# Eawag-SIAM/SimulatedAnnealingABC.jl

Hardware: AMD Instinct MI355X
Metric: particle-simulations/sec at n_particles=1e6 (higher is better)
Workload: dtype f64

## Files before the change

### include/sabc_hip.h

```cpp
#ifndef SABC_HIP_H
#define SABC_HIP_H

#include <stdint.h>

#ifdef __cplusplus
extern "C" {
#endif

#define SABC_ABI_VERSION 6
#define SABC_MAX_PARA 16
#define SABC_MAX_STATS 64
#define SABC_MAX_SOURCE_STATS 64
#define SABC_MAX_JOINT_PARA 8
#define SABC_MAX_MODEL_PARAMS 32

#if defined(__GNUC__)
#define SABC_API __attribute__((visibility("default")))
#else
#define SABC_API
#endif

enum { SABC_MODEL_HOST = 0,
       SABC_MODEL_GAUSS_IID = 1, SABC_MODEL_GAUSS2D = 2, SABC_MODEL_GK = 3, SABC_MODEL_LV = 4,
       SABC_MODEL_USER = 5     };
// ... 115 lines not shown
SABC_API int64_t     sabc_comm_p2p_fallbacks(const sabc_handle *h);
SABC_API int         sabc_comm_p2p_inject_silence(sabc_handle *h, int32_t n);
SABC_API int         sabc_comm_p2p_inject_loss(sabc_handle *h, int32_t n);
SABC_API int         sabc_comm_p2p_inject_stale(sabc_handle *h, int32_t n);

SABC_API int sabc_initialize(sabc_handle *h, int64_t n_simulation);
SABC_API int sabc_update(sabc_handle *h, const sabc_update_args *args);

SABC_API int64_t sabc_n_global(const sabc_handle *h);
SABC_API int64_t sabc_n_local(const sabc_handle *h);
SABC_API int64_t sabc_local_offset(const sabc_handle *h);
SABC_API int sabc_get_population(sabc_handle *h, double *theta, double *u, double *rho);
SABC_API int sabc_set_population(sabc_handle *h, const double *theta, const double *u, const double *rho);
SABC_API int sabc_get_counters(const sabc_handle *h, int64_t out[4]);
SABC_API int sabc_set_counters(sabc_handle *h, const int64_t in[4]);
SABC_API int sabc_get_epsilon(const sabc_handle *h, double *eps, int32_t *len);
SABC_API int sabc_set_epsilon(sabc_handle *h, const double *eps, int32_t len);
SABC_API int64_t sabc_history_len(const sabc_handle *h);
SABC_API int sabc_get_history(const sabc_handle *h, double *eps_hist, double *u_hist, double *rho_hist);
SABC_API int sabc_clear_history(sabc_handle *h);
SABC_API int64_t sabc_cdf_len(const sabc_handle *h, int32_t stat);
SABC_API int sabc_get_cdf_knots(sabc_handle *h, int32_t stat, double *out);
SABC_API int sabc_set_cdf_knots(sabc_handle *h, int32_t stat, const double *knots, int64_t len);
SABC_API int sabc_cdf_apply(sabc_handle *h, const double *rho, int64_t m, double *u_out);
SABC_API int sabc_get_proposal_sigma(const sabc_handle *h, double *sigma_dxd);
SABC_API double sabc_last_ess(const sabc_handle *h);

SABC_API int sabc_op_build_cdf(int32_t device, const double *x, int64_t n, double *knots_out, int64_t *len_out);
SABC_API int sabc_op_cdf_eval(int32_t device, const double *knots, int64_t len, const double *q, int64_t m,
                              double *out);
SABC_API int sabc_op_sort(int32_t device, const double *x, int64_t n, double *out);
SABC_API int sabc_op_eps_single(double ubar, double v, double *eps_out);
SABC_API int sabc_op_eps_multi(const double *ubar, int32_t s, double v, double *eps_out);
SABC_API int sabc_op_simulate(sabc_handle *h, const double *theta, int64_t m, uint64_t pid0, uint64_t iter,
                              double *rho_out);
SABC_API int sabc_op_prior(sabc_handle *h, uint64_t pid0, int64_t m, double *theta_out, double *logpdf_out);
SABC_API int sabc_op_philox(int32_t device, uint64_t seed, uint64_t pid, uint32_t purpose, uint64_t iter, uint32_t k,
                            uint32_t out_words[4], double out_normals[2]);

SABC_API int sabc_op_normal_pairs(int32_t device, uint64_t seed, uint64_t pid0, uint32_t purpose, uint64_t iter,
                                  uint32_t k, int64_t m, double *out_2m);

SABC_API int sabc_op_rng_peak(int32_t device, int64_t n_lanes, int32_t pairs_per_lane, int32_t repeats,
                              double *normals_per_s);

enum { SABC_KERNEL_UPDATE = 0, SABC_KERNEL_REDUCE = 1, SABC_KERNEL_RESAMPLE = 2, SABC_KERNEL_INIT = 3,
       SABC_KERNEL_COLLECTIVE = 4,
       SABC_KERNEL_COUNT = 5 };
SABC_API int sabc_profile_enable(sabc_handle *h, int32_t level);
SABC_API int sabc_profile_get(sabc_handle *h, int32_t kernel, double *total_ms, int64_t *launches);
SABC_API int64_t sabc_profile_noops(sabc_handle *h, int32_t kernel);
SABC_API int64_t sabc_host_syncs(const sabc_handle *h);
SABC_API int64_t sabc_kernel_launches(const sabc_handle *h);
SABC_API int64_t sabc_persistent_launches(const sabc_handle *h);
SABC_API int32_t sabc_persistent_lanes(const sabc_handle *h);
SABC_API int64_t sabc_persistent_fallbacks(const sabc_handle *h);
SABC_API int64_t sabc_collective_calls(const sabc_handle *h);

#ifdef __cplusplus
}
#endif
#endif
```

### simulatedannealingabc.jl_amd/_lib.py

```python
from __future__ import annotations

import ctypes as C
import os
import subprocess

_HERE = os.path.dirname(os.path.abspath(__file__))
CSRC = os.path.join(_HERE, "csrc")
LIB_PATH = os.path.join(_HERE, "libsabc_hip.so")
HEADER = os.path.normpath(os.path.join(_HERE, "..", "include", "sabc_hip.h"))

ABI_VERSION = 6
P2P_DESC_BYTES, P2P_MAX_WORLD = 512, 8
MAX_PARA, MAX_STATS, MAX_MODEL_PARAMS = 16, 64, 32
MAX_SOURCE_STATS = 64
MAX_JOINT_PARA = 8
MODEL_HOST, MODEL_GAUSS_IID, MODEL_GAUSS2D, MODEL_GK, MODEL_LV, MODEL_USER = 0, 1, 2, 3, 4, 5
PRIOR_NORMAL, PRIOR_UNIFORM, PRIOR_EXPONENTIAL, PRIOR_LOGNORMAL, PRIOR_GAMMA, PRIOR_BETA, PRIOR_TRUNCNORMAL = 0, 1, 2, 3, 4, 5, 6
PROP_RANDOMWALK, PROP_DIFFEVO, PROP_STRETCH = 0, 1, 2
ALG_SINGLE_EPS, ALG_MULTI_EPS = 0, 1
KERNEL_UPDATE, KERNEL_REDUCE, KERNEL_RESAMPLE, KERNEL_INIT, KERNEL_COLLECTIVE = 0, 1, 2, 3, 4

ERR_NAMES = {
    -1: "NSIM_TOO_SMALL", -2: "NEG_DISTANCE", -3: "BAD_V", -4: "BAD_DELTA", -5: "BAD_ALGORITHM", -6: "BAD_BETA",
    -7: "ZERO_MEAN_U", -8: "BAD_CONFIG", -9: "NOT_POSDEF", -10: "EMPTY_CDF", -11: "ROOT", -20: "NO_DEVICE",
# ... 100 lines not shown
        "sabc_last_error": ([vp], C.c_char_p),
        "sabc_set_stream": ([vp, vp], C.c_int),
        "sabc_set_collectives": ([vp, ALLREDUCE_FN, ALLGATHER_FN, vp, C.c_int], C.c_int),
        "sabc_set_alltoallv": ([vp, ALLTOALLV_FN], C.c_int),
        "sabc_comm_bytes": ([vp], C.c_int64),
        "sabc_set_host_simulator": ([vp, SIMULATE_FN, vp], C.c_int),
        "sabc_set_host_prior": ([vp, PRIOR_SAMPLE_FN, PRIOR_LOGPDF_FN, vp], C.c_int),
        "sabc_register_device_simulator": ([vp, C.c_char_p], C.c_int),
        "sabc_op_compile_device_simulator": ([C.c_char_p, C.c_int32, C.c_int32, C.c_char_p, C.c_int64], C.c_int),
        "sabc_op_compile_device_simulator_with_prior": ([C.c_char_p, C.c_int32, C.c_int32, C.c_char_p, C.c_int64], C.c_int),
        "sabc_comm_init_rccl": ([vp, vp], C.c_int),
        "sabc_comm_unique_id": ([vp], C.c_int),
        "sabc_comm_selftest": ([vp], C.c_int),
        "sabc_initialize": ([vp, C.c_int64], C.c_int),
        "sabc_update": ([vp, C.POINTER(UpdateArgs)], C.c_int),
        "sabc_n_global": ([vp], C.c_int64),
        "sabc_n_local": ([vp], C.c_int64),
        "sabc_local_offset": ([vp], C.c_int64),
        "sabc_get_population": ([vp, dp, dp, dp], C.c_int),
        "sabc_set_population": ([vp, dp, dp, dp], C.c_int),
        "sabc_get_counters": ([vp, ip64], C.c_int),
        "sabc_set_counters": ([vp, ip64], C.c_int),
        "sabc_get_epsilon": ([vp, dp, C.POINTER(C.c_int32)], C.c_int),
        "sabc_set_epsilon": ([vp, dp, C.c_int32], C.c_int),
        "sabc_history_len": ([vp], C.c_int64),
        "sabc_get_history": ([vp, dp, dp, dp], C.c_int),
        "sabc_clear_history": ([vp], C.c_int),
        "sabc_cdf_len": ([vp, C.c_int32], C.c_int64),
        "sabc_get_cdf_knots": ([vp, C.c_int32, dp], C.c_int),
        "sabc_set_cdf_knots": ([vp, C.c_int32, dp, C.c_int64], C.c_int),
        "sabc_cdf_apply": ([vp, dp, C.c_int64, dp], C.c_int),
        "sabc_get_proposal_sigma": ([vp, dp], C.c_int),
        "sabc_last_ess": ([vp], C.c_double),
        "sabc_op_build_cdf": ([C.c_int32, dp, C.c_int64, dp, ip64], C.c_int),
        "sabc_op_sort": ([C.c_int32, dp, C.c_int64, dp], C.c_int),
        "sabc_op_cdf_eval": ([C.c_int32, dp, C.c_int64, dp, C.c_int64, dp], C.c_int),
        "sabc_op_eps_single": ([C.c_double, C.c_double, dp], C.c_int),
        "sabc_op_eps_multi": ([dp, C.c_int32, C.c_double, dp], C.c_int),
        "sabc_op_simulate": ([vp, dp, C.c_int64, C.c_uint64, C.c_uint64, dp], C.c_int),
        "sabc_op_prior": ([vp, C.c_uint64, C.c_int64, dp, dp], C.c_int),
        "sabc_op_philox": ([C.c_int32, C.c_uint64, C.c_uint64, C.c_uint32, C.c_uint64, C.c_uint32,
                            C.POINTER(C.c_uint32), dp], C.c_int),
        "sabc_op_normal_pairs": ([C.c_int32, C.c_uint64, C.c_uint64, C.c_uint32, C.c_uint64, C.c_uint32, C.c_int64, dp],
                                 C.c_int),
        "sabc_op_rng_peak": ([C.c_int32, C.c_int64, C.c_int32, C.c_int32, dp], C.c_int),
        "sabc_profile_enable": ([vp, C.c_int32], C.c_int),
        "sabc_profile_get": ([vp, C.c_int32, dp, ip64], C.c_int),
        "sabc_profile_noops": ([vp, C.c_int32], C.c_int64),
        "sabc_set_host_chunk": ([vp, C.c_int64], C.c_int),
        "sabc_host_callback_seconds": ([vp], C.c_double),
        "sabc_host_callback_calls": ([vp], C.c_int64),
        "sabc_host_syncs": ([vp], C.c_int64),
        "sabc_kernel_launches": ([vp], C.c_int64),
        "sabc_persistent_launches": ([vp], C.c_int64),
        "sabc_persistent_lanes": ([vp], C.c_int32),
        "sabc_persistent_fallbacks": ([vp], C.c_int64),
        "sabc_collective_calls": ([vp], C.c_int64),
        "sabc_comm_p2p_setup": ([vp], C.c_int),
        "sabc_comm_p2p_descriptor": ([vp, vp], C.c_int),
        "sabc_comm_p2p_init": ([vp, vp], C.c_int),
        "sabc_comm_p2p_selftest": ([vp], C.c_int),
        "sabc_comm_p2p_set_timeout": ([vp, C.c_double], C.c_int),
        "sabc_comm_p2p_disable": ([vp], C.c_int),
        "sabc_comm_p2p_active": ([vp], C.c_int),
        "sabc_comm_p2p_fallbacks": ([vp], C.c_int64),
        "sabc_comm_p2p_inject_silence": ([vp, C.c_int32], C.c_int),
        "sabc_comm_p2p_inject_stale": ([vp, C.c_int32], C.c_int),
        "sabc_comm_p2p_inject_loss": ([vp, C.c_int32], C.c_int),
        "sabc_comm_p2p_set_destroy_wait": ([vp, C.c_double], C.c_int),
        "sabc_comm_p2p_parked_bytes": ([], C.c_int64),
    }
    for name, (args, res) in sig.items():
        if not strict and not hasattr(L, name):
            continue
        fn = getattr(L, name)
        fn.argtypes, fn.restype = args, res
    return L


def global_error() -> str:
    return lib().sabc_last_global_error().decode("utf-8", "replace")
```

### simulatedannealingabc.jl_amd/csrc/capi.hip

```cpp
#include <hip/hip_runtime.h>
#include <dlfcn.h>

#include <cstdio>
#include <cstdlib>
#include <cstring>
#include <mutex>
#include <new>
#include <string>
#include <vector>

#include "../../include/sabc_hip.h"
#include "engine.hpp"
#include "hip_backend.hpp"
#include "host_math.hpp"
#include "kernels.hpp"
#include "p2p.hpp"
#include "p2p_setup.hpp"
#include "rtc.hpp"

using namespace sabc;

namespace {

thread_local std::string g_err;
// ... 622 lines not shown
  if (e == hipSuccess) e = hipMalloc((void **)&z, 16);
  if (e == hipSuccess) e = (hipError_t)launch_philox_debug(seed, pid, purpose, iter, k, w, z, nullptr);
  if (e == hipSuccess) e = hipMemcpy(out_words, w, 16, hipMemcpyDeviceToHost);
  if (e == hipSuccess) e = hipMemcpy(out_normals, z, 16, hipMemcpyDeviceToHost);
  (void)hipFree(w); (void)hipFree(z);
  if (e != hipSuccess) { g_err = hipGetErrorString(e); return SABC_ERR_HIP; }
  return 0;
}

int sabc_op_normal_pairs(int32_t device, uint64_t seed, uint64_t pid0, uint32_t purpose, uint64_t iter, uint32_t k,
                         int64_t m, double *out_2m) {
  std::string why;
  int rc = usable_device(device, why);
  if (rc) { g_err = why; return rc; }
  if (m <= 0) return 0;
  if (hipSetDevice(device) != hipSuccess) { g_err = "hipSetDevice failed"; return SABC_ERR_HIP; }
  double *d = nullptr;
  hipError_t e = hipMalloc((void **)&d, (size_t)m * 16);
  if (e == hipSuccess) e = (hipError_t)launch_normal_pairs(seed, pid0, purpose, iter, k, m, d, nullptr);
  if (e == hipSuccess) e = hipMemcpy(out_2m, d, (size_t)m * 16, hipMemcpyDeviceToHost);
  (void)hipFree(d);
  if (e != hipSuccess) { g_err = hipGetErrorString(e); return SABC_ERR_HIP; }
  return 0;
}

int sabc_op_rng_peak(int32_t device, int64_t n_lanes, int32_t pairs_per_lane, int32_t repeats, double *normals_per_s) {
  std::string why;
  int rc = usable_device(device, why);
  if (rc) { g_err = why; return rc; }
  if (n_lanes < 1 || pairs_per_lane < 1 || repeats < 1) { g_err = "bad arguments"; return SABC_ERR_BAD_CONFIG; }
  if (hipSetDevice(device) != hipSuccess) { g_err = "hipSetDevice failed"; return SABC_ERR_HIP; }
  double *d = nullptr;
  hipEvent_t a = nullptr, b = nullptr;
  hipError_t e = hipMalloc((void **)&d, (size_t)n_lanes * 8);
  if (e == hipSuccess) e = hipEventCreate(&a);
  if (e == hipSuccess) e = hipEventCreate(&b);
  if (e == hipSuccess) e = (hipError_t)launch_rng_peak(1, pairs_per_lane, n_lanes, d, nullptr);
  if (e == hipSuccess) e = hipEventRecord(a, nullptr);
  for (int r = 0; r < repeats && e == hipSuccess; ++r) e = (hipError_t)launch_rng_peak(2 + r, pairs_per_lane, n_lanes, d, nullptr);
  if (e == hipSuccess) e = hipEventRecord(b, nullptr);
  if (e == hipSuccess) e = hipEventSynchronize(b);
  float ms = 0.f;
  if (e == hipSuccess) e = hipEventElapsedTime(&ms, a, b);
  if (a) (void)hipEventDestroy(a);
  if (b) (void)hipEventDestroy(b);
  (void)hipFree(d);
  if (e != hipSuccess) { g_err = hipGetErrorString(e); return SABC_ERR_HIP; }
  *normals_per_s = 2.0 * (double)pairs_per_lane * (double)n_lanes * (double)repeats / ((double)ms * 1e-3);
  return 0;
}

int64_t sabc_host_syncs(const sabc_handle *h) { return h ? h->eng->host_syncs() : 0; }
int64_t sabc_kernel_launches(const sabc_handle *h) { return h ? h->be->kernel_launches() : 0; }
int64_t sabc_collective_calls(const sabc_handle *h) { return h ? h->eng->collective_calls() : 0; }

int sabc_profile_enable(sabc_handle *h, int32_t on) {
  if (!h) return SABC_ERR_STATE;
  h->be->profile_enable(on);
  return 0;
}

int64_t sabc_profile_noops(sabc_handle *h, int32_t kernel) { return h ? h->be->profile_noops(kernel) : 0; }

int sabc_profile_get(sabc_handle *h, int32_t kernel, double *total_ms, int64_t *launches) {
  if (!h) return SABC_ERR_STATE;
  return h->be->profile_get(kernel, total_ms, launches) ? hfail(h, SABC_ERR_HIP) : 0;
}

}
```

### simulatedannealingabc.jl_amd/csrc/device_models.hpp

```cpp
#pragma once
#include "device_rng.hpp"
#include "prior_math.hpp"
#include "kernels.hpp"
#include "sabc_types.hpp"

#ifndef SABC_GK_BLOCKMAX
#define SABC_GK_BLOCKMAX 1
#endif

namespace sabc {

#define SABC_LOG2PI 1.8378770664093454835606594728112

__device__ __forceinline__ double prior_logpdf_dim(const ModelDesc &m, int k, double x) {
  const int kind = m.prior_kind[k];
  const double a = m.prior_a[k], b = m.prior_b[k], lc = m.prior_logc[k];
  if (kind == SABC_PRIOR_NORMAL) {
    const double z = (x - a) / b;
    return -(z * z + SABC_LOG2PI) / 2.0 - lc;
  }
  if (kind == SABC_PRIOR_UNIFORM) return (x >= a && x <= b) ? -lc : -INFINITY;
  if (kind == SABC_PRIOR_EXPONENTIAL) return x >= 0.0 ? -x / a - lc : -INFINITY;
  if (kind == SABC_PRIOR_LOGNORMAL) {
    if (!(x > 0.0)) return -INFINITY;
// ... 302 lines not shown
  return cdf_interp(T, len, lo, x);
}

template <int N>
__device__ __forceinline__ void cdf_apply_mid_lockstep(const double *__restrict__ T, int64_t len, const double *__restrict__ M,
                                                       const double *x, double *u) {
  const int64_t mcount = (len + 15) >> kCdfLineShift;
  int64_t top = 1;
  while (top < mcount) top <<= 1;
  int64_t a[N];
#pragma unroll
  for (int p = 0; p < N; ++p) a[p] = 0;
  for (int64_t step = top >> 1; step >= 1; step >>= 1) {
#pragma unroll
    for (int p = 0; p < N; ++p) {
      const int64_t q = a[p] + step;
      const int64_t qs = q < mcount ? q : mcount - 1;
      const double v = M[qs];
      a[p] = (q < mcount && v < x[p]) ? q : a[p];
    }
  }
#pragma unroll
  for (int p = 0; p < N; ++p) a[p] <<= kCdfLineShift;
#pragma unroll
  for (int step = 1 << kCdfLineShift >> 1; step >= 1; step >>= 1) {
#pragma unroll
    for (int p = 0; p < N; ++p) a[p] += (T[a[p] + step] < x[p]) ? step : 0;
  }
  const double first = T[0], last = T[len - 1], L1 = (double)(len - 1);
  double t0[N], t1[N];
  int64_t i0[N];
#pragma unroll
  for (int p = 0; p < N; ++p) {
    const int64_t lo = first < x[p] ? a[p] + 1 : 0;
    i0[p] = lo > 0 ? lo - 1 : 0;
    t0[p] = T[i0[p]]; t1[p] = T[i0[p] + 1];
  }
#pragma unroll
  for (int p = 0; p < N; ++p) {
    const double y0 = (double)i0[p] / L1, y1 = (double)(i0[p] + 1) / L1;
    const double t = (x[p] - t0[p]) / (t1[p] - t0[p]);
    const double v = y0 + t * (y1 - y0);
    u[p] = !(x[p] >= first) ? ((x[p] != x[p]) ? x[p] : 0.0) : (x[p] > last ? 1.0 : v);
  }
}

__device__ __forceinline__ double finite_or_big(double v) { return isfinite(v) ? v : 1e30; }

template <int MODEL, int D, int S>
struct Sim;

template <int D, int S>
struct Sim<SABC_MODEL_GAUSS_IID, D, S> {
  static __device__ __forceinline__ void run(const ModelDesc &m, const double *th, uint64_t pid, uint64_t iter,
                                             double *rho, int coop = 0) {
    const int n_obs = (int)m.p[0];
    const double mu = th[0];
    const double sd = (D >= 2) ? th[1] : m.p[1];
    NormalStream ns(m.seed, pid, PURPOSE_SIM, iter, coop);
    double sz = 0.0, szz = 0.0;
    const int n_pairs = n_obs >> 1;
    ns.for_pairs(n_pairs, [&](const double z0, const double z1) {
      sz += z0; if (S >= 2) szz = fma(z0, z0, szz);
      sz += z1; if (S >= 2) szz = fma(z1, z1, szz);
    });
    if (n_obs & 1) {
      double z0, z1;
      ns.pair(z0, z1);
      sz += z0; if (S >= 2) szz = fma(z0, z0, szz);
    }
    const double n = (double)n_obs;
    rho[0] = fabs(m.p[2] - (mu + sd * sz / n));
    if (S >= 2) rho[1] = fabs(m.p[3] - (mu * mu + (2.0 * mu * sd * sz + sd * sd * szz) / n));
  }
};

template <int D, int S>
struct Sim<SABC_MODEL_GAUSS2D, D, S> {
  static __device__ __forceinline__ void run(const ModelDesc &m, const double *th, uint64_t pid, uint64_t iter,
                                             double *rho, int coop = 0) {
    const int n_obs = (int)m.p[0];
    const double r = m.p[1], c = sqrt(1.0 - r * r);
    NormalStream ns(m.seed, pid, PURPOSE_SIM, iter, coop);
    double A = 0, B = 0, AA = 0, BB = 0, AB = 0;
    ns.for_pairs(n_obs, [&](const double za, const double zb) {
      A += za; B += zb; AA = fma(za, za, AA); BB = fma(zb, zb, BB); AB = fma(za, zb, AB);
    });
    const double S1 = A, S2 = r * A + c * B;
    const double Q11 = AA, Q22 = r * r * AA + 2.0 * r * c * AB + c * c * BB, Q12 = r * AA + c * AB;
    const double m1 = S1 / n_obs, m2 = S2 / n_obs;
    const double var1 = (Q11 - S1 * m1) / (n_obs - 1), var2 = (Q22 - S2 * m2) / (n_obs - 1);
    const double cov = (Q12 - S1 * m2) / (n_obs - 1);
    const double d1 = th[0] + m1 - m.p[2], d2 = th[1] + m2 - m.p[3];
    rho[0] = sqrt(d1 * d1 + d2 * d2);
    if (S >= 2) rho[1] = fabs(var1 + var2 - m.p[4]);
    if (S >= 3) rho[2] = fabs(cov - m.p[5]);
  }
};

#if !defined(__HIPCC_RTC__)
constexpr int kGkMaxDraws = 128;
#ifndef SABC_GK_PW
#define SABC_GK_PW 64
#endif
constexpr int kGkParticlesPerWave = SABC_GK_PW;

__device__ __forceinline__ double gk_quantile(const double *th, double c, double z) {
  const double w = exp_tab(-0.5 * th[3] * neg2_log_tab(fma(z, z, 1.0)));
  return th[0] + th[1] * (1.0 + c * tanh_abs_tab(th[2] * z / 2.0)) * w * z;
}

template <int DIST>
__device__ __forceinline__ double xor_lane(double v) {
  int lo = __double2loint(v), hi = __double2hiint(v);
  if constexpr (DIST == 1) {
    lo = __builtin_amdgcn_mov_dpp(lo, 0xB1, 0xF, 0xF, true);
    hi = __builtin_amdgcn_mov_dpp(hi, 0xB1, 0xF, 0xF, true);
  } else if constexpr (DIST == 2) {
    lo = __builtin_amdgcn_mov_dpp(lo, 0x4E, 0xF, 0xF, true);
    hi = __builtin_amdgcn_mov_dpp(hi, 0x4E, 0xF, 0xF, true);
  } else if constexpr (DIST <= 16) {
    constexpr int pattern = 0x1F | (DIST << 10);
    lo = __builtin_amdgcn_ds_swizzle(lo, pattern);
    hi = __builtin_amdgcn_ds_swizzle(hi, pattern);
  } else {
    return __shfl_xor(v, DIST, 64);
  }
  return __hiloint2double(hi, lo);
}

template <int DIST>
__device__ __forceinline__ void half_swap(double &a, double &b) {
  static_assert(DIST == 16 || DIST == 32, "row-pair or half-wave swap");
  unsigned alo = (unsigned)__double2loint(a), ahi = (unsigned)__double2hiint(a);
  unsigned blo = (unsigned)__double2loint(b), bhi = (unsigned)__double2hiint(b);
  if constexpr (DIST == 32) {
    const auto l = __builtin_amdgcn_permlane32_swap(alo, blo, false, false);
    const auto h = __builtin_amdgcn_permlane32_swap(ahi, bhi, false, false);
    alo = l[0]; blo = l[1]; ahi = h[0]; bhi = h[1];
  } else {
    const auto l = __builtin_amdgcn_permlane16_swap(alo, blo, false, false);
    const auto h = __builtin_amdgcn_permlane16_swap(ahi, bhi, false, false);
    alo = l[0]; blo = l[1]; ahi = h[0]; bhi = h[1];
  }
  a = __hiloint2double((int)ahi, (int)alo);
  b = __hiloint2double((int)bhi, (int)blo);
}

constexpr uint64_t lane_bit(int i) {
// ... 171 lines not shown
  for (int i = 0; i < 8; ++i) v[i] = __hiloint2double(__double2hiint(v[i]) ^ sign_mask, __double2loint(v[i]));
}

template <int S>
__device__ __forceinline__ void gk_simulate_rows4(const ModelDesc &m, const double (*thp_lds)[4], double (*rp_lds)[S], const int my,
                                                  const uint64_t pid, const uint64_t iter) {
  const int lane = threadIdx.x & 63, rl = lane & 15;
  const int n_draws = (int)m.p[0];
  const double c = m.p[1];
  double th[4];
#pragma unroll
  for (int k = 0; k < 4; ++k) th[k] = thp_lds[my][k];
  const bool inc = gk_increasing(th, c);
  double v[8];
#pragma unroll
  for (int t = 0; t < 4; ++t) box_muller(stream_block(m.seed, pid, PURPOSE_SIM, iter, (uint32_t)(4 * rl + t)), v[2 * t], v[2 * t + 1]);
  if (!inc) {
#pragma unroll
    for (int i = 0; i < 8; ++i) v[i] = gk_quantile(th, c, v[i]);
  }
#pragma unroll
  for (int i = 0; i < 8; ++i) v[i] = 8 * rl + i < n_draws ? v[i] : INFINITY;
  const int b0 = (lane & 1) << 31, b1 = (lane & 2) << 30, b2 = (lane & 4) << 29, b3 = (lane & 8) << 28;
  gk_local_step<0, 1>(v);
  gk_local_step<1, 2>(v); gk_local_step<0, 2>(v);
  gk_flip(v, b0);
  gk_local_step<2, -1>(v); gk_local_step<1, -1>(v); gk_local_step<0, -1>(v);
  gk_flip(v, b1); gk_cross_step<1>(v);
  gk_flip(v, b0); gk_local_step<2, -1>(v); gk_local_step<1, -1>(v); gk_local_step<0, -1>(v);
  gk_flip(v, b2); gk_cross_step<2>(v);
  gk_flip(v, b1 ^ b0); gk_cross_step<1>(v);
  gk_flip(v, b0); gk_local_step<2, -1>(v); gk_local_step<1, -1>(v); gk_local_step<0, -1>(v);
  gk_flip(v, b3); gk_cross_step<4>(v);
  gk_flip(v, b2 ^ b1); gk_cross_step<2>(v);
  gk_flip(v, b1 ^ b0); gk_cross_step<1>(v);
  gk_flip(v, b0); gk_local_step<2, -1>(v); gk_local_step<1, -1>(v); gk_local_step<0, -1>(v);
  gk_cross_step<8>(v);
  gk_flip(v, b3 ^ b2); gk_cross_step<4>(v);
  gk_flip(v, b2 ^ b1); gk_cross_step<2>(v);
  gk_flip(v, b1);
  double bm = gk_max(gk_max(gk_max(v[0], v[1]), gk_max(v[2], v[3])), gk_max(gk_max(v[4], v[5]), gk_max(v[6], v[7])));
  bm = gk_max(bm, xor_lane<1>(bm));
#pragma unroll
  for (int j = 0; j < S; ++j) {
    const int lane_of_block = (((int)m.p[2 + j] >> 4) - 1) * 2;
    if (rl == lane_of_block) rp_lds[my][j] = inc ? bm : finite_or_big(fabs(bm - m.p[2 + S + j]));
  }
}

#endif

template <int D, int S>
struct Sim<SABC_MODEL_LV, D, S> {
  static __device__ __forceinline__ void run(const ModelDesc &m, const double *th, uint64_t pid, uint64_t iter,
                                             double *rho, int coop = 0) {
    const int n_steps = (int)m.p[0];
    const double dt = m.p[1], sg = m.p[2];
    double X = m.p[3], Y = m.p[4];
    const double sdt = sg * sqrt(dt);
    NormalStream ns(m.seed, pid, PURPOSE_SIM, iter, coop);
    double SX = 0, QX = 0, SY = 0, QY = 0;
    ns.for_pairs(n_steps, [&](const double z1, const double z2) {
      const double fx = fma(sdt, z1, fma(-th[1], Y, th[0]) * dt);
      const double fy = fma(sdt, z2, fma(th[1], X, -th[2]) * dt);
      X = fmax(fma(X, fx, X), 0.0);
      Y = fmax(fma(Y, fy, Y), 0.0);
      SX += X; QX += X * X; SY += Y; QY += Y * Y;
    });
    const double mX = SX / n_steps, mY = SY / n_steps;
    const double vX = (QX - SX * mX) / (n_steps - 1), vY = (QY - SY * mY) / (n_steps - 1);
    const double st[4] = {mX, sqrt(fmax(vX, 0.0)), mY, sqrt(fmax(vY, 0.0))};
#pragma unroll
    for (int j = 0; j < S; ++j) rho[j] = finite_or_big(fabs(st[j < 4 ? j : 3] - m.p[5 + j]));
  }
};

}
```

### simulatedannealingabc.jl_amd/csrc/device_rng.hpp

```cpp
#pragma once
#if !defined(__HIPCC_RTC__)
#include <hip/hip_runtime.h>
#endif
#include <stdint.h>
#ifndef INFINITY
#define INFINITY (__builtin_huge_val())
#endif

namespace sabc {

enum : uint32_t { PURPOSE_PRIOR = 0, PURPOSE_SIM = 1, PURPOSE_PROP = 2, PURPOSE_PROP2 = 3, PURPOSE_ACCEPT = 4,
                  PURPOSE_RESAMPLE = 5 };

struct u32x4 { uint32_t x, y, z, w; };

#if defined(__has_builtin)
#if __has_builtin(__builtin_amdgcn_bitop3_b32) && !defined(SABC_NO_BITOP3)
#define SABC_HAVE_BITOP3 1
#endif
#endif
__device__ __forceinline__ uint32_t xor3(uint32_t a, uint32_t b, uint32_t c) {
#if defined(SABC_HAVE_BITOP3)
  return __builtin_amdgcn_bitop3_b32(a, b, c, 0x96);
#else
// ... 260 lines not shown
}

__device__ __forceinline__ void box_muller(const u32x4 w, double &z0, double &z1, const Regs &c) {
  const double ua = loop::u52(w.x, w.y, c);
  const double ub = loop::u52(w.z, w.w, c);
  const double r = sqrt_fast(loop::neg2_log_tab(ua));
  double sn, cs;
  loop::sincos_2pi_tab(ub, sn, cs, c);
  z0 = r * cs;
  z1 = r * sn;
}

}

template <int W, int J>
__device__ __forceinline__ double team_pick_ct(const double v) {
  static_assert((W == 4 || W == 16) && J >= 0 && J < W, "a quad or a row of 16 lanes");
  constexpr int ctrl = W == 4 ? J * 0x55 : 0x150 + J;
  const int lo = __builtin_amdgcn_update_dpp(0, __double2loint(v), ctrl, 0xF, 0xF, true);
  const int hi = __builtin_amdgcn_update_dpp(0, __double2hiint(v), ctrl, 0xF, 0xF, true);
  return __hiloint2double(hi, lo);
}
template <int W, int J0 = 0, int N = W>
__device__ __forceinline__ double team_pick(const double v, const uint32_t j) {
  if constexpr (N == 1) {
    return team_pick_ct<W, J0>(v);
  } else {
    return (j & (uint32_t)(N / 2)) ? team_pick<W, J0 + N / 2, N / 2>(v, j) : team_pick<W, J0, N / 2>(v, j);
  }
}

#ifndef SABC_SIM_UNROLL
#define SABC_SIM_UNROLL 2
#endif

constexpr int kCoopPlainLoop = -1;

template <int... J> struct lane_seq {};
template <int N, int... J> struct make_lane_seq : make_lane_seq<N - 1, N - 1, J...> {};
template <int... J> struct make_lane_seq<0, J...> { using type = lane_seq<J...>; };

struct NormalStream {
  uint64_t seed, pid, iter;
  uint32_t purpose, k;
  double spare;
  bool have;
  int coop;
  int buf_block;
  bool buf_uniform;
  double b0, b1;
  __device__ __forceinline__ NormalStream(uint64_t seed_, uint64_t pid_, uint32_t purpose_, uint64_t iter_, int coop_ = 0)
      : seed(seed_), pid(pid_), iter(iter_), purpose(purpose_), k(0), spare(0.0), have(false), coop(coop_), buf_block(-1),
        buf_uniform(false), b0(0.0), b1(0.0) {}
  __device__ __forceinline__ void pair(double &z0, double &z1) {
    if (coop == 4) { fetch<4>(k++, false, z0, z1); return; }
    if (coop == 16) { fetch<16>(k++, false, z0, z1); return; }
    box_muller(stream_block(seed, pid, purpose, iter, k++), z0, z1);
  }
  __device__ __forceinline__ void uniform_pair(double &u0, double &u1) {
    if (coop == 4) { fetch<4>(k++, true, u0, u1); return; }
    if (coop == 16) { fetch<16>(k++, true, u0, u1); return; }
    const u32x4 w = stream_block(seed, pid, purpose, iter, k++);
    u0 = u52(w.x, w.y);
    u1 = u52(w.z, w.w);
  }
  template <class F>
  __device__ __forceinline__ void for_pairs(const int n, F &&f) {
    if (coop == 0) { for_pairs_lane(n, f); return; }
    for_pairs_plain(n, f);
  }
  __device__ __forceinline__ double next() {
    if (have) { have = false; return spare; }
    double z0;
    pair(z0, spare);
    have = true;
    return z0;
  }

 private:
  template <class F>
  __device__ __forceinline__ void for_pairs_lane(const int n, F &f) {
    const loop::Regs c = loop::Regs::load();
#pragma unroll SABC_SIM_UNROLL
    for (int i = 0; i < n; ++i) {
      double z0, z1;
      loop::box_muller(loop::stream_block(seed, pid, purpose, iter, k++), z0, z1, c);
      f(z0, z1);
    }
  }
  template <class F>
  __device__ __forceinline__ void for_pairs_plain(const int n, F &&f) {
    if (coop == 4) { for_pairs_team<4>(n, f); return; }
    if (coop == 16) { for_pairs_team<16>(n, f); return; }
#pragma unroll SABC_SIM_UNROLL
    for (int i = 0; i < n; ++i) {
      double z0, z1;
      pair(z0, z1);
      f(z0, z1);
    }
  }
  template <int W, class F, int... J>
  __device__ __forceinline__ void hand_out(const double g0, const double g1, F &f, lane_seq<J...>) {
    (f(team_pick_ct<W, J>(g0), team_pick_ct<W, J>(g1)), ...);
  }
  template <int W, class F, int... J>
  __device__ __forceinline__ void hand_out_first(const int m, const double g0, const double g1, F &f, lane_seq<J...>) {
// ... 51 lines not shown
```

### simulatedannealingabc.jl_amd/csrc/hip_backend.hip

```cpp
#include "hip_backend.hpp"

#include <hip/hip_runtime.h>
#include <unistd.h>
#include <atomic>
#include <chrono>
#include <cmath>
#include <string>
#include <cstdio>
#include <cstdlib>
#include <cstring>

namespace sabc {

namespace {
std::atomic<int64_t> g_parked_bytes{0};
}

#define HB_CHECK(expr, what)                       \
  do {                                             \
    const int rc_ = check((expr), (what));         \
    if (rc_) return rc_;                           \
  } while (0)

#define HB_LAUNCH(expr, what)                      \
  do {                                             \
    (void)hipGetLastError();                       \
    const int e_ = (expr);                         \
    launches_ += 1;                                \
    if (e_) return check((hipError_t)e_, (what));  \
  } while (0)

static double persist_timeout_ms() {
  const char *e = std::getenv("SABC_PERSISTENT_TIMEOUT_MS");
  const double v = e ? std::atof(e) : 0.0;
  return v > 0 ? v : 2000.0;
}

namespace {
std::mutex g_stream_pool_mutex;
std::vector<std::pair<int, hipStream_t>> *g_stream_pool = nullptr;
constexpr size_t kStreamPoolMax = 32;

hipStream_t pooled_stream_take(int device) {
  std::lock_guard<std::mutex> lock(g_stream_pool_mutex);
  if (!g_stream_pool) return nullptr;
  for (size_t i = 0; i < g_stream_pool->size(); ++i)
    if ((*g_stream_pool)[i].first == device) {
      hipStream_t s = (*g_stream_pool)[i].second;
      g_stream_pool->erase(g_stream_pool->begin() + (long)i);
      return s;
    }
  return nullptr;
}
void pooled_stream_give(int device, hipStream_t s) {
  if (hipStreamSynchronize(s) != hipSuccess) { (void)hipGetLastError(); (void)hipStreamDestroy(s); return; }
  std::lock_guard<std::mutex> lock(g_stream_pool_mutex);
  if (!g_stream_pool) g_stream_pool = new std::vector<std::pair<int, hipStream_t>>();
  if (g_stream_pool->size() >= kStreamPoolMax) { (void)hipStreamDestroy(s); return; }
  g_stream_pool->emplace_back(device, s);
}
}

static double persist_rendezvous_ms() {
  const char *e = std::getenv("SABC_PERSISTENT_RENDEZVOUS_MS");
  const double v = e ? std::atof(e) : 0.0;
  return v > 0 ? v : 20.0;
}

HipBackend::HipBackend(int device) : device_(device) {
  if (const char *e = std::getenv("SABC_PERSISTENT_MAX")) persist_max_ = std::atoll(e);
  if (const char *e = std::getenv("SABC_PERSISTENT")) { if (e[0] == '0') persist_max_ = 0; }
  if (const char *e = std::getenv("SABC_FUSE_REDUCE_MAX")) {
    const long long v = std::atoll(e);
    if (v >= 0) fuse_reduce_max_ = v;
  }
}

void HipBackend::free_later(void *p) {
  if (p) deferred_free_.push_back(p);
}

void HipBackend::end_of_call() {
  for (void *p : deferred_free_) (void)hipFree(p);
  deferred_free_.clear();
}

HipBackend::~HipBackend() {
  if (!stream_ && !pop_[0]) return;
  (void)hipSetDevice(device_);
  if (stream_) (void)hipStreamSynchronize(stream_);
  const size_t pop_bytes = (size_t)(m_.d + m_.s + 1) * (size_t)sh_.cap * sizeof(double), rho_bytes = (size_t)m_.s * (size_t)sh_.cap * sizeof(double);
  if (!p2p_finish()) {
    g_parked_bytes += (int64_t)((pop_[0] ? pop_bytes : 0) + (pop_[1] ? pop_bytes : 0) + (rho_ ? rho_bytes : 0) + (slots_ ? (size_t)kP2PSlotWords * 8 : 0));
    pop_[0] = pop_[1] = rho_ = nullptr;
    slots_ = nullptr;
  }
  end_of_call();
  for (auto &v : ev_)
    for (auto &e : v) { (void)hipEventDestroy(e.a); (void)hipEventDestroy(e.b); }
  for (auto &e : ev_pool_) { (void)hipEventDestroy(e.a); (void)hipEventDestroy(e.b); }
  double *dev[] = {pop_[0], pop_[1], rho_, knots_, coarse_, mid_, partials_, hist_dev_, sums_stage_, gather_, cum_, block_sums_, totals_dev_, col_a_, col_b_, pack_dev_};
  for (double *p : dev)
    if (p) (void)hipFree(p);
  for (double *p : scratch_)
    if (p) (void)hipFree(p);
  if (idx_dev_) (void)hipFree(idx_dev_);
  if (slot_dev_) (void)hipFree(slot_dev_);
  if (bucket_dev_) (void)hipFree(bucket_dev_);
  if (bucket_host_) (void)hipHostFree(bucket_host_);
  double *staged[] = {host_thp_, host_rho_, host_cur_, host_lp2_};
  for (double *p : staged)
    if (p) (void)hipHostFree(p);
  if (host_gate_) (void)hipHostFree(host_gate_);
  if (dev_thp_) (void)hipFree(dev_thp_);
  if (dev_aux_) (void)hipFree(dev_aux_);
  if (dev_rho_prop_) (void)hipFree(dev_rho_prop_);
  if (host_flag_) (void)hipHostFree(host_flag_);
  if (host_done_dev_) (void)hipFree(host_done_dev_);
  if (host_acc_dev_) (void)hipFree(host_acc_dev_);
  if (sort_tmp_) (void)hipFree(sort_tmp_);
  if (meta_dev_) (void)hipFree(meta_dev_);
  if (cb_dev_) (void)hipFree(cb_dev_);
  if (pinned_block_) (void)hipHostFree(pinned_block_);
  rtc_release(&rtc_);
  if (persist_sync_) (void)hipFree(persist_sync_);
  if (persist_rows_) (void)hipFree(persist_rows_);
  if (slots_) (void)hipFree(slots_);
  if (p2p_test_dev_) (void)hipFree(p2p_test_dev_);
  if (snap_pop_) (void)hipFree(snap_pop_);
  if (snap_rho_) (void)hipFree(snap_rho_);
  if (own_stream_ && stream_) pooled_stream_give(device_, stream_);
}

int HipBackend::check(hipError_t e, const char *what) {
  if (e == hipSuccess) return 0;
  char buf[256];
  std::snprintf(buf, sizeof(buf), "HIP error %d (%s) in %s", (int)e, hipGetErrorString(e), what);
  err_ = buf;
  return -1;
}

int HipBackend::set_stream(hipStream_t s) {
  HB_CHECK(hipSetDevice(device_), "hipSetDevice");
  if (stream_) HB_CHECK(hipStreamSynchronize(stream_), "hipStreamSynchronize");
  if (own_stream_ && stream_) pooled_stream_give(device_, stream_);
  stream_ = s;
  own_stream_ = false;
  return 0;
}

PopPtrs HipBackend::pop_ptrs(int which) const {
  PopPtrs pp;
  pp.pop = pop_[which];
  pp.rho = rho_;
  pp.cap = sh_.cap;
  pp.n_local = sh_.n_local;
  pp.gid0 = sh_.gid0;
  return pp;
}

CdfPtrs HipBackend::cdf_ptrs() const {
  CdfPtrs c;
  c.knots = knots_;
  c.stride = knot_stride_;
  c.coarse = coarse_;
  c.mid = mid_;
  c.mid_stride = mid_stride_;
  for (int j = 0; j < kMaxStats; ++j) { c.len[j] = cdf_len_[j]; c.shift[j] = cdf_shift_[j]; }
  return c;
}

int HipBackend::allocate(const ModelDesc &m, const Shard &sh) {
  m_ = m;
  sh_ = sh;
  np_ = n_partials(m.d, m.s);
  HB_CHECK(hipSetDevice(device_), "hipSetDevice");
  if (!stream_) {
    stream_ = pooled_stream_take(device_);
    if (!stream_) HB_CHECK(hipStreamCreateWithFlags(&stream_, hipStreamNonBlocking), "hipStreamCreate");
    own_stream_ = true;
  }
  const size_t cap = (size_t)sh.cap, N = (size_t)sh.n_global;
  const size_t rows = (size_t)(m.d + m.s + 1);
  static const bool fine = [] { const char *e = std::getenv("SABC_P2P_FINEGRAINED"); return !(e && e[0] == '0'); }();
  auto pop_alloc = [&](double **p, size_t bytes) {
    return fine && sh.world > 1 ? hipExtMallocWithFlags((void **)p, bytes, hipDeviceMallocFinegrained) : hipMalloc((void **)p, bytes);
  };
  for (int b = 0; b < 2; ++b) {
    HB_CHECK(pop_alloc(&pop_[b], rows * cap * sizeof(double)), "hipMalloc(pop)");
    HB_CHECK(hipMemsetAsync(pop_[b], 0, rows * cap * sizeof(double), stream_), "hipMemset(pop)");
  }
  HB_CHECK(pop_alloc(&rho_, (size_t)m.s * cap * sizeof(double)), "hipMalloc(rho)");
  HB_CHECK(hipMemsetAsync(rho_, 0, (size_t)m.s * cap * sizeof(double), stream_), "hipMemset(rho)");
  HB_CHECK(hipMalloc((void **)&coarse_, (size_t)m.s * cdf_coarse_entries(m.s) * sizeof(double)), "hipMalloc(coarse)");
  knot_stride_ = (((int64_t)N + 2 + 15) / 16) * 16 + 16;
  HB_CHECK(hipMalloc((void **)&knots_, (size_t)m.s * (size_t)knot_stride_ * sizeof(double)), "hipMalloc(knots)");
  mid_stride_ = cdf_mid_stride(knot_stride_);
  HB_CHECK(hipMalloc((void **)&mid_, (size_t)m.s * (size_t)mid_stride_ * sizeof(double)), "hipMalloc(mid)");
  {
    const int64_t per_half = update_rows(m, (sh.cap + 1) / 2) + 1, whole = update_rows(m, sh.cap);
    partial_rows_ = 2 * per_half > whole ? 2 * per_half : whole;
    if (partial_rows_ < n_blocks(sh.cap)) partial_rows_ = n_blocks(sh.cap);
    if (2 * persistent_workgroups_bound(m, sh.cap) > partial_rows_) partial_rows_ = 2 * persistent_workgroups_bound(m, sh.cap);
    partial_rows_ += 4;
  }
  HB_CHECK(hipMalloc((void **)&partials_, (size_t)partial_rows_ * np_ * sizeof(double)), "hipMalloc(partials)");
  HB_CHECK(hipMalloc((void **)&cb_dev_, sizeof(ControlBlock)), "hipMalloc(control block)");
  HB_CHECK(hipMemsetAsync(cb_dev_, 0, sizeof(ControlBlock), stream_), "hipMemset(control block)");
  {
    const size_t off_mbox = (sizeof(ControlBlock) + 255) / 256 * 256, off_totals = off_mbox + (kMailboxRing * sizeof(Mailbox) + 255) / 256 * 256;
    HB_CHECK(hipHostMalloc((void **)&pinned_block_, off_totals + 256, hipHostMallocMapped), "hipHostMalloc(control block, mailbox, totals)");
    char *pinned_dev = nullptr;
    HB_CHECK(hipHostGetDevicePointer((void **)&pinned_dev, pinned_block_, 0), "hipHostGetDevicePointer(pinned block)");
    cb_host_ = reinterpret_cast<ControlBlock *>(pinned_block_);
    mbox_host_ = reinterpret_cast<Mailbox *>(pinned_block_ + off_mbox);
    mbox_dev_ = reinterpret_cast<Mailbox *>(pinned_dev + off_mbox);
    totals_host_ = reinterpret_cast<double *>(pinned_block_ + off_totals);
    totals_host_dev_ = reinterpret_cast<double *>(pinned_dev + off_totals);
  }
  HB_CHECK(hipMalloc((void **)&sums_stage_, kMaxPartials * sizeof(double)), "hipMalloc(sums staging)");
  HB_CHECK(hipMemsetAsync(sums_stage_, 0, kMaxPartials * sizeof(double), stream_), "hipMemset(sums staging)");
  for (int i = 0; i < kMailboxRing; ++i) { mbox_host_[i].w0 = kMailboxEmpty; mbox_host_[i].w1 = kMailboxEmpty; }
  HB_CHECK(hipMalloc((void **)&cum_, N * sizeof(double)), "hipMalloc(cum)");
  HB_CHECK(hipMalloc((void **)&block_sums_, (size_t)weight_scan_doubles((int64_t)N) * sizeof(double)), "hipMalloc(block_sums)");
  HB_CHECK(hipMalloc((void **)&totals_dev_, 2 * sizeof(double)), "hipMalloc(totals)");
  totals_host_[0] = totals_host_[1] = 0.0;
  HB_CHECK(hipMalloc((void **)&meta_dev_, 2 * kMaxStats * sizeof(int64_t)), "hipMalloc(meta)");
  int khz = 0;
  if (hipDeviceGetAttribute(&khz, hipDeviceAttributeWallClockRate, device_) == hipSuccess && khz > 0) wall_clock_khz_ = khz;
  else (void)hipGetLastError();
  return 0;
}

double *HipBackend::gather_buffer(int64_t doubles) {
  if (doubles > gather_cap_) {
    if (stream_) (void)hipStreamSynchronize(stream_);
    free_later(gather_);
    gather_ = nullptr;
    gather_cap_ = 0;
    if (hipMalloc((void **)&gather_, (size_t)doubles * sizeof(double)) != hipSuccess) return nullptr;
    gather_cap_ = doubles;
  }
  return gather_;
}

double *HipBackend::scratch_buffer(int which, int64_t doubles) {
  if (which < 0 || which >= 4) return nullptr;
  if (doubles > scratch_cap_[which]) {
    if (stream_) (void)hipStreamSynchronize(stream_);
    free_later(scratch_[which]);
    scratch_[which] = nullptr;
    scratch_cap_[which] = 0;
    const int64_t want = doubles + doubles / 4 + 64;
    if (hipMalloc((void **)&scratch_[which], (size_t)want * sizeof(double)) != hipSuccess) return nullptr;
    scratch_cap_[which] = want;
  }
  return scratch_[which];
}

int HipBackend::copy_rows(const double *src, int64_t src_pitch, double *dst, int64_t dst_pitch, int rows, int64_t count) {
  if (rows <= 0 || count <= 0) return 0;
  HB_CHECK(hipMemcpy2DAsync(dst, (size_t)dst_pitch * sizeof(double), src, (size_t)src_pitch * sizeof(double),
                            (size_t)count * sizeof(double), (size_t)rows, hipMemcpyDeviceToDevice, stream_), "copy_rows");
  return 0;
}

int HipBackend::to_backend(double *dst, const double *src_host, int64_t n) {
  if (n <= 0) return 0;
  HB_CHECK(hipMemcpyAsync(dst, src_host, (size_t)n * sizeof(double), hipMemcpyHostToDevice, stream_), "to_backend");
  HB_CHECK(hipStreamSynchronize(stream_), "hipStreamSynchronize");
  return 0;
}

int HipBackend::to_host(double *dst_host, const double *src, int64_t n) {
  if (n <= 0) return 0;
  HB_CHECK(hipMemcpyAsync(dst_host, src, (size_t)n * sizeof(double), hipMemcpyDeviceToHost, stream_), "to_host");
  HB_CHECK(hipStreamSynchronize(stream_), "hipStreamSynchronize");
  return 0;
}

// ... 216 lines not shown
        double *dst = host_thv_.data() + (size_t)k * mv;
        for (int64_t i = 0; i < mv; ++i) dst[i] = src[host_where_[(size_t)i]];
      }
      th_arg = host_thv_.data(); rho_arg = host_rhov_.data();
    }
    if (mv > 0) {
      const auto c0 = std::chrono::steady_clock::now();
      const int rc = host_fn_(host_ctx_, th_arg, host_ids_.data(), mv, c.iter, rho_arg);
      host_cb_seconds_ += std::chrono::duration<double>(std::chrono::steady_clock::now() - c0).count();
      host_cb_calls_ += 1;
      if (rc) { err_ = "the host simulator (f_dist) failed"; return -1; }
    }
    if (!direct)
      for (int j = 0; j < s; ++j) {
        double *dst = host_rho_ + (size_t)j * cnt;
        for (int64_t t = 0; t < tn; ++t) dst[t0 + t] = 0.0;
        const double *src = host_rhov_.data() + (size_t)j * mv;
        for (int64_t i = 0; i < mv; ++i) dst[host_where_[(size_t)i]] = src[i];
      }
    if (ch == 0) prof_begin(SABC_KERNEL_UPDATE);
    HB_LAUNCH(launch_host_accept(m_, c, cb_dev_, pop_ptrs(cur_), cdf_ptrs(), lo, cnt, t0, tn, dev_thp_, dev_aux_, host_rho_dev_,
                                 host_prior ? host_lp2_dev_ : nullptr, host_acc_dev_, stream_), "k_host_accept");
    if (ch == n_chunks - 1) prof_end(SABC_KERNEL_UPDATE);
  }
  return 0;
}

int HipBackend::host_stats(int64_t *rows_out) {
  if (ensure_host_buffers()) return -1;
  HB_LAUNCH(launch_stats_rt(m_, cb_dev_, pop_ptrs(cur_), partials_, host_acc_dev_, stream_), "k_stats_rt");
  *rows_out = n_blocks(sh_.n_local);
  return 0;
}

int HipBackend::register_device_simulator(const char *hip_source) {
  if (m_.model_id != SABC_MODEL_USER) { err_ = "the handle was not created with SABC_MODEL_USER"; return -1; }
  HB_CHECK(hipSetDevice(device_), "hipSetDevice");
  if (stream_) HB_CHECK(hipStreamSynchronize(stream_), "hipStreamSynchronize");
  rtc_release(&rtc_);
  std::string log;
  const bool small = persist_max_ > 0 && sh_.world == 1 && sh_.n_local <= persist_max_ && persistent_fits(m_.d, m_.s);
  if (rtc_build(hip_source, m_.d, m_.s, rtc_default_csrc_dir(), &rtc_, &log, m_.prior_joint == 3, small)) {
    std::string log_chain;
    if (!small || rtc_build(hip_source, m_.d, m_.s, rtc_default_csrc_dir(), &rtc_, &log_chain, m_.prior_joint == 3, false)) {
      err_ = "compiling the device simulator failed:\n" + log;
      return -1;
    }
  }
  return 0;
}

int HipBackend::prior_simulate() {
  if (m_.model_id == SABC_MODEL_USER && !rtc()) { err_ = "no device simulator registered (sabc_register_device_simulator)"; return -1; }
  prof_begin(SABC_KERNEL_INIT);
  HB_LAUNCH(launch_prior_simulate(m_, pop_ptrs(cur_), stream_, rtc()), "k_prior_simulate");
  prof_end(SABC_KERNEL_INIT);
  return 0;
}

int HipBackend::build_cdf(const double *gathered_rho, int64_t *len_out, int *any_negative) {
  return build_cdf_blocks(flat_blocks(gathered_rho, m_.s, sh_.cap, sh_.world), len_out, any_negative);
}

int HipBackend::build_cdf_blocks(const ShardBlocks &rho_blocks, int64_t *len_out, int *any_negative) {
  const int64_t N = sh_.n_global;
  if (!col_a_) {
    HB_CHECK(hipMalloc((void **)&col_a_, (size_t)N * sizeof(double)), "hipMalloc(col_a)");
    HB_CHECK(hipMalloc((void **)&col_b_, (size_t)N * sizeof(double)), "hipMalloc(col_b)");
    size_t bytes = 0;
    HB_LAUNCH(sort_f64(col_a_, col_b_, N, nullptr, &bytes, stream_), "radix sort size query");
    sort_tmp_bytes_ = bytes ? bytes : 16;
    HB_CHECK(hipMalloc(&sort_tmp_, sort_tmp_bytes_), "hipMalloc(sort_tmp)");
  }
  for (int j = 0; j < m_.s; ++j) {
    HB_LAUNCH(launch_compact_column(rho_blocks, j, N, col_a_, stream_), "k_compact_column");
    size_t bytes = sort_tmp_bytes_;
    HB_LAUNCH(sort_f64(col_a_, col_b_, N, sort_tmp_, &bytes, stream_), "radix sort");
    launches_ += 31;
    HB_LAUNCH(launch_cdf_knots(col_b_, N, knots_ + (int64_t)j * knot_stride_, meta_dev_ + 2 * j, stream_), "k_cdf_knots");
    launches_ += 1;
  }
  int64_t meta[2 * kMaxStats];
  HB_CHECK(hipMemcpyAsync(meta, meta_dev_, 2 * (size_t)m_.s * sizeof(int64_t), hipMemcpyDeviceToHost, stream_), "memcpy(meta)");
  HB_CHECK(hipStreamSynchronize(stream_), "hipStreamSynchronize");
  *any_negative = 0;
  for (int j = 0; j < m_.s; ++j) {
    const int64_t mpos = N - meta[2 * j];
    cdf_len_[j] = mpos > 0 ? mpos + 2 : 0;
    len_out[j] = cdf_len_[j];
    if (meta[2 * j + 1]) *any_negative = 1;
    if (cdf_len_[j] > 0 && build_coarse(j)) return -1;
  }
  free_later(col_a_); free_later(col_b_); free_later(sort_tmp_);
  col_a_ = col_b_ = nullptr; sort_tmp_ = nullptr;
  return 0;
}

int HipBackend::cdf_population() {
  HB_LAUNCH(launch_cdf_population(m_, pop_ptrs(cur_), cdf_ptrs(), stream_), "k_cdf_population");
  return 0;
}

int HipBackend::update_range(const StepArgs &c, const PartnerView &pv, int64_t lo, int64_t cnt, int64_t row0,
                             int64_t *rows_out) {
  const int64_t rows = update_rows(m_, cnt);
  if (lo < 0 || cnt < 0 || lo + cnt > sh_.n_local || row0 + rows > partial_rows_) {
    err_ = "update_range: range outside the shard";
    return -1;
  }
  hipEvent_t ev0 = nullptr, ev1 = nullptr;
  if (prof_ && (prof_ != 1 || (prof_tick_++ & 1) == 0)) {
    EvPair e{nullptr, nullptr};
    if (!ev_pool_.empty()) { e = ev_pool_.back(); ev_pool_.pop_back(); }
    else if (hipEventCreate(&e.a) != hipSuccess || hipEventCreate(&e.b) != hipSuccess) e = EvPair{nullptr, nullptr};
    if (e.a && e.b) { ev_[SABC_KERNEL_UPDATE].push_back(e); ev0 = e.a; ev1 = e.b; }
  }
  HB_LAUNCH(launch_update(m_, c, cb_dev_, pop_ptrs(cur_), cdf_ptrs(), pv, lo, cnt, partials_, row0, stream_, ev0, ev1, rtc()), "k_update");
  *rows_out = rows;
  return 0;
}

bool HipBackend::persistent_supported(int prop_kind) const {
  if (persist_max_ <= 0 || sh_.world != 1 || sh_.n_local > persist_max_ || prof_ >= 2) return false;
  const int64_t wg = persistent_workgroups(m_, prop_kind, sh_.n_local, rtc());
  return wg > 0 && 2 * wg <= partial_rows_;
}

int HipBackend::update_persistent(const StepArgs &c, const ControlArgs &ctrl, const PartnerView &pv_a, const PartnerView &pv_b, int64_t ix0,
                                  int64_t phase, int64_t cph, int64_t count, int64_t *done, int *halted, int *error) {
  if (pending_rows_ >= 0 && flush_reduce()) return -1;
  if (!persist_sync_) HB_CHECK(hipMalloc((void **)&persist_sync_, 4 * sizeof(unsigned long long)), "hipMalloc(grid barrier)");
  HB_CHECK(hipMemsetAsync(persist_sync_, 0, 4 * sizeof(unsigned long long), stream_), "hipMemset(grid barrier)");
  PersistArgs pa;
  std::memset(&pa, 0, sizeof(pa));
  pa.iter0 = c.iter;
  pa.ix0 = ix0; pa.phase = phase; pa.cph = cph;
  pa.act_n = sh_.n_local; pa.half = sh_.n_local / 2;
  pa.count = (int32_t)(count > (int64_t)1 << 30 ? (int64_t)1 << 30 : count);
  pa.prop_p0 = c.prop_p0; pa.prop_p1 = c.prop_p1;
  pa.ctrl = ctrl;
  pa.sync = persist_sync_;
  pa.timeout_ticks = (uint64_t)(persist_timeout_ms() * (double)wall_clock_khz_);
  pa.rendezvous_ticks = (uint64_t)(persist_rendezvous_ms() * (double)wall_clock_khz_);
  if (const char *e = std::getenv("SABC_PERSISTENT_TEST_ABSENT_WG")) pa.test_absent_wg = std::atoi(e);
  const int64_t wg = persistent_workgroups(m_, c.prop_kind, pa.act_n, rtc(), &persist_lanes_);
  if (wg <= 0) return check(hipErrorInvalidValue, "k_update_persistent: no one-launch form for this shard");
  const size_t row_bytes = (size_t)np_ * 2 * sizeof(unsigned long long);
  if (!persist_rows_ || persist_rows_wg_ < wg) {
    if (persist_rows_) (void)hipFree(persist_rows_);
    persist_rows_ = nullptr;
    persist_rows_wg_ = persistent_workgroups_bound(m_, sh_.cap) > wg ? persistent_workgroups_bound(m_, sh_.cap) : wg;
    HB_CHECK(hipMalloc((void **)&persist_rows_, 2 * (size_t)persist_rows_wg_ * row_bytes), "hipMalloc(partial rows of the one-launch form)");
  }
  HB_CHECK(hipMemsetAsync(persist_rows_, 0, 2 * (size_t)wg * row_bytes, stream_), "hipMemset(partial rows of the one-launch form)");
  prof_begin(SABC_KERNEL_UPDATE);
  HB_LAUNCH(launch_update_persistent(m_, c.prop_kind, pa, cb_dev_, pop_ptrs(cur_), cdf_ptrs(), pv_a, pv_b, reinterpret_cast<double *>(persist_rows_),
                                     hist_dev_, mbox_dev_, sums_stage_, stream_, rtc()), "k_update_persistent");
  prof_end(SABC_KERNEL_UPDATE);
  ControlBlock cb;
  if (read_control(&cb)) return -1;
  *done = cb.persist_done;
  *halted = cb.halt;
  *error = cb.error;
  return 0;
}

int HipBackend::stats(int64_t *rows_out) {
  HB_LAUNCH(launch_stats(m_, cb_dev_, pop_ptrs(cur_), partials_, stream_, rtc()), "k_stats");
  *rows_out = n_blocks(sh_.n_local);
  return 0;
}

int HipBackend::reduce_partials(int64_t rows, bool guarded) {
  if (pending_rows_ >= 0 && flush_reduce()) return -1;
  pending_rows_ = rows;
  pending_guarded_ = guarded;
  return 0;
}

int HipBackend::flush_reduce() {
  if (pending_rows_ < 0) return 0;
  const int64_t rows = pending_rows_;
  pending_rows_ = -1;
  prof_begin(SABC_KERNEL_REDUCE);
  HB_LAUNCH(launch_reduce_partials(partials_, rows, np_, sums_stage_, pending_guarded_ ? &cb_dev_->halt : nullptr, stream_),
            "k_reduce_partials");
  if (pending_xchg_) {
    pending_xchg_ = false;
    ControlArgs none;
    std::memset(&none, 0, sizeof(none));
    none.mode = pending_guarded_ ? CTRL_GUARDED : 0;
    const P2PView pv = p2p_view();
    HB_LAUNCH(launch_reduce_control(partials_, -1, np_, sums_stage_, pending_guarded_, cb_dev_, none, hist_dev_, mbox_dev_, stream_, &pv,
                                    tag(++xseq_), false, take_silence()), "k_reduce_control (exchange)");
  }
  prof_end(SABC_KERNEL_REDUCE);
  return 0;
}

double *HipBackend::sums_buffer() {
  (void)flush_reduce();
  return sums_stage_;
}

int HipBackend::control(const ControlArgs &a) {
  const bool xchg = pending_xchg_ && pending_rows_ >= 0;
  const P2PView pv = xchg ? p2p_view() : P2PView();
  if (pending_rows_ >= 0 && np_ <= 64 && pending_rows_ * np_ <= fuse_reduce_max_) {
    const int64_t rows = pending_rows_;
    pending_rows_ = -1;
    pending_xchg_ = false;
    prof_begin(SABC_KERNEL_REDUCE);
    HB_LAUNCH(launch_reduce_control(partials_, rows, np_, sums_stage_, pending_guarded_, cb_dev_, a, hist_dev_, mbox_dev_, stream_,
                                    xchg ? &pv : nullptr, xchg ? tag(++xseq_) : 0, true, xchg ? take_silence() : 0),
              "k_reduce_control");
    prof_end(SABC_KERNEL_REDUCE);
    return 0;
  }
  if (xchg) {
    pending_xchg_ = false;
    if (flush_reduce()) return -1;
    prof_begin(SABC_KERNEL_REDUCE);
    HB_LAUNCH(launch_reduce_control(partials_, -1, np_, sums_stage_, pending_guarded_, cb_dev_, a, hist_dev_, mbox_dev_, stream_, &pv,
                                    tag(++xseq_), true, take_silence()), "k_reduce_control (exchange)");
    prof_end(SABC_KERNEL_REDUCE);
    return 0;
  }
  if (flush_reduce()) return -1;
  HB_LAUNCH(launch_control(cb_dev_, a, hist_dev_, mbox_dev_, sums_stage_, stream_), "k_control");
  return 0;
}

int HipBackend::wait_notify(int64_t seq, int64_t *n_accept, int *error, int *halted) {
  Mailbox *mb = mbox_host_ + (seq % kMailboxRing);
  int32_t e = 0, hl = 0;
  for (uint64_t spins = 1;; ++spins) {
    if (mailbox_unpack(mb->w0, mb->w1, seq, n_accept, &e, &hl)) break;
    __builtin_ia32_pause();
    if ((spins & 0x3FFF) == 0) {
      const hipError_t q = hipStreamQuery(stream_);
      if (q == hipSuccess) {
        if (mailbox_unpack(mb->w0, mb->w1, seq, n_accept, &e, &hl)) break;
        err_ = "control step did not report back although the stream is idle";
        return -1;
      }
      if (q != hipErrorNotReady) return check(q, "hipStreamQuery");
    }
  }
  *error = (int)e;
  *halted = (int)hl;
  return 0;
}

int HipBackend::read_control(ControlBlock *out) {
  HB_CHECK(hipMemcpyAsync(cb_host_, cb_dev_, sizeof(ControlBlock), hipMemcpyDeviceToHost, stream_), "memcpy(control block)");
  HB_CHECK(hipStreamSynchronize(stream_), "hipStreamSynchronize");
  std::memcpy(out, cb_host_, sizeof(ControlBlock));
  return 0;
}

int HipBackend::write_control(const ControlBlock &in) {
  HB_CHECK(hipStreamSynchronize(stream_), "hipStreamSynchronize");
  std::memcpy(cb_host_, &in, sizeof(ControlBlock));
  HB_CHECK(hipMemcpyAsync(cb_dev_, cb_host_, sizeof(ControlBlock), hipMemcpyHostToDevice, stream_), "memcpy(control block)");
  return 0;
}

// ... 69 lines not shown
            "k_resample_select");
  prof_end(SABC_KERNEL_RESAMPLE);
  return 0;
}

int HipBackend::resample_bucket(int64_t *counts_host, double *req_out) {
  const int W = sh_.world;
  const size_t bytes = (size_t)W * sizeof(unsigned long long);
  HB_CHECK(hipMemsetAsync(bucket_dev_, 0, 2 * bytes, stream_), "hipMemset(buckets)");
  HB_LAUNCH(launch_bucket_count(idx_dev_, sh_.n_local, sh_.cap, bucket_dev_, stream_), "k_bucket_count");
  HB_CHECK(hipMemcpyAsync(bucket_host_, bucket_dev_, bytes, hipMemcpyDeviceToHost, stream_), "memcpy(bucket counts)");
  HB_CHECK(hipStreamSynchronize(stream_), "hipStreamSynchronize");
  unsigned long long run = 0;
  for (int r = 0; r < W; ++r) {
    counts_host[r] = (int64_t)bucket_host_[r];
    bucket_host_[W + r] = run;
    run += bucket_host_[r];
  }
  if ((int64_t)run != sh_.n_local) { err_ = "resample_bucket: the bucket counts do not add up to n_local"; return -1; }
  HB_CHECK(hipMemcpyAsync(bucket_dev_ + W, bucket_host_ + W, bytes, hipMemcpyHostToDevice, stream_), "memcpy(bucket cursors)");
  HB_LAUNCH(launch_bucket_scatter(idx_dev_, sh_.n_local, sh_.cap, bucket_dev_ + W, req_out, slot_dev_, stream_), "k_bucket_scatter");
  return 0;
}

int HipBackend::resample_serve(const double *req_in, int64_t m, double *rows_out) {
  HB_LAUNCH(launch_resample_serve(req_in, m, m_.d + m_.s, pop_ptrs(cur_), rows_out, stream_), "k_resample_serve");
  return 0;
}

int HipBackend::resample_scatter(const double *rows_in) {
  const int nxt = 1 - cur_;
  HB_LAUNCH(launch_resample_scatter(rows_in, slot_dev_, sh_.n_local, m_.d + m_.s, pop_ptrs(nxt), stream_), "k_resample_scatter");
  flip_cur();
  return 0;
}

double HipBackend::last_ess() {
  if (stream_) (void)hipStreamSynchronize(stream_);
  return totals_host_ && totals_host_[1] > 0 ? totals_host_[0] * totals_host_[0] / totals_host_[1] : 0.0;
}

int HipBackend::download(double *theta, double *u, double *rho) {
  const size_t w = (size_t)sh_.n_local * sizeof(double), pitch = (size_t)sh_.cap * sizeof(double);
  if (sh_.n_local > 0) {
    if (theta) HB_CHECK(hipMemcpy2DAsync(theta, w, pop_[cur_], pitch, w, (size_t)m_.d, hipMemcpyDeviceToHost, stream_), "download theta");
    if (u) HB_CHECK(hipMemcpy2DAsync(u, w, pop_[cur_] + (size_t)m_.d * sh_.cap, pitch, w, (size_t)m_.s, hipMemcpyDeviceToHost, stream_), "download u");
    if (rho) HB_CHECK(hipMemcpy2DAsync(rho, w, rho_, pitch, w, (size_t)m_.s, hipMemcpyDeviceToHost, stream_), "download rho");
  }
  HB_CHECK(hipStreamSynchronize(stream_), "hipStreamSynchronize");
  return 0;
}

int HipBackend::upload(const double *theta, const double *u, const double *rho) {
  const size_t w = (size_t)sh_.n_local * sizeof(double), pitch = (size_t)sh_.cap * sizeof(double);
  if (sh_.n_local > 0) {
    if (theta) HB_CHECK(hipMemcpy2DAsync(pop_[cur_], pitch, theta, w, w, (size_t)m_.d, hipMemcpyHostToDevice, stream_), "upload theta");
    if (u) HB_CHECK(hipMemcpy2DAsync(pop_[cur_] + (size_t)m_.d * sh_.cap, pitch, u, w, w, (size_t)m_.s, hipMemcpyHostToDevice, stream_), "upload u");
    if (rho) HB_CHECK(hipMemcpy2DAsync(rho_, pitch, rho, w, w, (size_t)m_.s, hipMemcpyHostToDevice, stream_), "upload rho");
  }
  HB_CHECK(hipStreamSynchronize(stream_), "hipStreamSynchronize");
  return 0;
}

int HipBackend::get_knots(int stat, double *out, int64_t len) {
  if (stat < 0 || stat >= m_.s || len > cdf_len_[stat]) { err_ = "get_knots: bad statistic index or length"; return -1; }
  HB_CHECK(hipMemcpyAsync(out, knots_ + (int64_t)stat * knot_stride_, (size_t)len * sizeof(double), hipMemcpyDeviceToHost, stream_), "memcpy(knots)");
  HB_CHECK(hipStreamSynchronize(stream_), "hipStreamSynchronize");
  return 0;
}

int HipBackend::set_knots(int stat, const double *knots, int64_t len) {
  if (stat < 0 || stat >= m_.s || len < 3 || len > knot_stride_ - 16) { err_ = "set_knots: bad statistic index or length"; return -1; }
  for (int64_t i = 0; i < len; ++i) {
    if (!(std::isfinite(knots[i]) && knots[i] >= 0.0)) { err_ = "set_knots: knots must be finite and non-negative"; return -1; }
    if (i > 0 && knots[i] < knots[i - 1]) { err_ = "set_knots: knots must be non-decreasing"; return -1; }
  }
  HB_CHECK(hipMemcpyAsync(knots_ + (int64_t)stat * knot_stride_, knots, (size_t)len * sizeof(double), hipMemcpyHostToDevice, stream_), "memcpy(knots)");
  HB_CHECK(hipStreamSynchronize(stream_), "hipStreamSynchronize");
  cdf_len_[stat] = len;
  return build_coarse(stat);
}

int HipBackend::build_coarse(int stat) {
  int shift = 0;
  const int nc = cdf_coarse_entries(m_.s);
  while ((((int64_t)cdf_len_[stat] + ((int64_t)1 << shift) - 1) >> shift) > nc) ++shift;
  cdf_shift_[stat] = shift;
  HB_LAUNCH(launch_cdf_index(knots_ + (int64_t)stat * knot_stride_, cdf_len_[stat], knot_stride_, shift,
                             coarse_ + (int64_t)stat * nc, nc, mid_ + (int64_t)stat * mid_stride_, mid_stride_, stream_),
            "k_cdf_index");
  return 0;
}

int HipBackend::cdf_apply_host(const double *rho, int64_t m, double *u_out) {
  if (m <= 0) return 0;
  double *d_in = nullptr, *d_out = nullptr;
  const size_t bytes = (size_t)m * m_.s * sizeof(double);
  HB_CHECK(hipMalloc((void **)&d_in, bytes), "hipMalloc");
  HB_CHECK(hipMalloc((void **)&d_out, bytes), "hipMalloc");
  int rc = check(hipMemcpyAsync(d_in, rho, bytes, hipMemcpyHostToDevice, stream_), "memcpy");
  if (!rc) rc = check((hipError_t)launch_cdf_apply_matrix(cdf_ptrs(), m_.s, d_in, m, d_out, stream_), "k_cdf_apply_matrix");
  if (!rc) rc = check(hipMemcpyAsync(u_out, d_out, bytes, hipMemcpyDeviceToHost, stream_), "memcpy");
  if (!rc) rc = check(hipStreamSynchronize(stream_), "hipStreamSynchronize");
  (void)hipFree(d_in); (void)hipFree(d_out);
  return rc;
}
// ... 374 lines not shown
```

### simulatedannealingabc.jl_amd/csrc/hip_backend.hpp

```cpp
#pragma once
#include <hip/hip_runtime_api.h>
#include <string>
#include <mutex>
#include <utility>
#include <vector>
#include "engine.hpp"
#include "kernels.hpp"
#include "p2p_page.hpp"

namespace sabc {

class HipBackend : public Backend {
 public:
  explicit HipBackend(int device);
  ~HipBackend() override;

  int allocate(const ModelDesc &m, const Shard &sh) override;
  double *pop_block() override { return pop_[cur_]; }
  double *rho_block() override { return rho_; }
  double *sums_buffer() override;
  double *gather_buffer(int64_t doubles) override;
  double *scratch_buffer(int which, int64_t doubles) override;
  int copy_rows(const double *src, int64_t src_pitch, double *dst, int64_t dst_pitch, int rows, int64_t count) override;
  int to_backend(double *dst, const double *src_host, int64_t n) override;
// ... 14 lines not shown
                   int64_t *rows_out) override;
  bool persistent_supported(int prop_kind) const override;
  int persistent_lanes() const override { return persist_lanes_; }
  int update_persistent(const StepArgs &c, const ControlArgs &ctrl, const PartnerView &pv_a, const PartnerView &pv_b, int64_t ix0,
                        int64_t phase, int64_t cph, int64_t count, int64_t *done, int *halted, int *error) override;
  int stats(int64_t *rows_out) override;
  int reduce_partials(int64_t rows, bool guarded) override;
  int control(const ControlArgs &a) override;
  int wait_notify(int64_t seq, int64_t *n_accept, int *error, int *halted) override;
  int read_control(ControlBlock *out) override;
  int write_control(const ControlBlock &in) override;
  int history_reserve(int64_t rows) override;
  int read_history(double *out, int64_t rows, int row_len) override;
  int resample_weights(double delta) override;
  int resample_draw(const double *gathered_pop, uint64_t iter) override;
  int resample_local(double delta, uint64_t iter, int64_t *stats_rows) override;
  int resample_select(const double *gathered_w, uint64_t iter) override;
  int resample_bucket(int64_t *counts_host, double *req_out) override;
  int resample_serve(const double *req_in, int64_t m, double *rows_out) override;
  int resample_scatter(const double *rows_in) override;
  double last_ess() override;
  void end_of_call() override;
  void prof_begin(int kernel) override;
  void prof_end(int kernel) override;
  int64_t profile_noops(int kernel) const { return kernel >= 0 && kernel < SABC_KERNEL_COUNT ? prof_noop_[kernel] : 0; }
  int download(double *theta, double *u, double *rho) override;
  int upload(const double *theta, const double *u, const double *rho) override;
  int get_knots(int stat, double *out, int64_t len) override;
  int set_knots(int stat, const double *knots, int64_t len) override;

  bool p2p_active() const override { return p2p_on_; }
  int p2p_exchange_pending() override { pending_xchg_ = true; return 0; }
  int p2p_barrier(bool guarded) override;
  int p2p_commit(int status, bool wait) override;
  void p2p_disable() override { (void)p2p_leave(); }
  bool p2p_peers_present() override;
  int build_cdf_p2p(int64_t *len_out, int *any_negative) override;
  int partner_view_p2p(PartnerView *pv) override;
  int resample_p2p(double delta, uint64_t iter) override;
  int snapshot() override;
  int restore_snapshot() override;
  int p2p_descriptor(P2PDesc *out);
  int p2p_init(const P2PDesc *all);
  int p2p_selftest();
  int p2p_leave();
  void p2p_forget_export() { if (!mapped_) exported_ = false; }
  void p2p_set_destroy_wait(double ms) { destroy_wait_ms_ = ms; }
  void p2p_inject_stale(int n) { p2p_stale_ = n > 0 ? n : 0; }
  static int64_t parked_bytes();
  void p2p_set_timeout(double ms) { if (ms > 0) p2p_timeout_ms_ = ms; }
  void p2p_inject_silence(int n) { p2p_loss_ = false; if (n >= 0) { p2p_skip_ = 0; p2p_silent_ = n; } else { p2p_skip_ = -n; p2p_silent_ = 1; } }
  void p2p_inject_loss(int n) { p2p_loss_ = true; p2p_skip_ = n > 0 ? n : 0; p2p_silent_ = 1; }
  int64_t kernel_launches() const { return launches_; }
  double host_callback_seconds() const { return host_cb_seconds_; }
  int64_t host_callback_calls() const { return host_cb_calls_; }
  void set_host_chunk(int64_t particles) { host_chunk_ = particles > 0 ? particles : 0; }

  int set_stream(hipStream_t s);
  hipStream_t stream() const { return stream_; }
  int device() const { return device_; }
  const std::string &error() const { return err_; }
  CdfPtrs cdf_ptrs() const;
  void set_cdf_len(int stat, int64_t len) { cdf_len_[stat] = len; }
  int cdf_apply_host(const double *rho, int64_t m, double *u_out);
  int simulate_host(const double *theta, int64_t n, uint64_t pid0, uint64_t iter, double *rho_out);
  int prior_host(uint64_t pid0, int64_t n, double *theta_out, double *logpdf_out);
  void profile_enable(int level);
  int profile_get(int kernel, double *total_ms, int64_t *launches);
  double *host_stage(int64_t doubles);

 private:
  int check(hipError_t e, const char *what);
  PopPtrs pop_ptrs(int which) const;

  int device_ = 0;
  hipStream_t stream_ = nullptr;
  bool own_stream_ = false;
  char *pinned_block_ = nullptr;
  std::string err_;
  ModelDesc m_{};
  Shard sh_{};
  int np_ = 0;
  double *pop_[2] = {nullptr, nullptr};
  int cur_ = 0;
  double *rho_ = nullptr, *knots_ = nullptr, *coarse_ = nullptr, *mid_ = nullptr;
  int64_t mid_stride_ = 0;
  int32_t cdf_shift_[kMaxStats] = {0};
  int build_coarse(int stat);
  int64_t knot_stride_ = 0;
  int64_t cdf_len_[kMaxStats] = {0};
  double *partials_ = nullptr;
  int64_t partial_rows_ = 0;
  ControlBlock *cb_dev_ = nullptr, *cb_host_ = nullptr;
  Mailbox *mbox_host_ = nullptr, *mbox_dev_ = nullptr;
  double *hist_dev_ = nullptr;
  int flush_reduce();
  int64_t pending_rows_ = -1;
  int64_t fuse_reduce_max_ = kFuseReduceMaxDoubles;
  bool pending_guarded_ = false;
  double *sums_stage_ = nullptr;
  int64_t hist_cap_ = 0;
  double *gather_ = nullptr;
  int64_t gather_cap_ = 0;
  double *scratch_[4] = {nullptr, nullptr, nullptr, nullptr};
  int64_t scratch_cap_[4] = {0, 0, 0, 0};
  int64_t *idx_dev_ = nullptr, *slot_dev_ = nullptr;
// ... 22 lines not shown
  unsigned int *host_done_dev_ = nullptr;
  unsigned long long host_seq_ = 0;
  int64_t host_chunk_ = 0;
  std::vector<int64_t> host_ids_, host_where_;
  std::vector<double> host_thv_, host_rhov_, host_both_, host_lp_;
  double host_cb_seconds_ = 0.0;
  int64_t host_cb_calls_ = 0;
  unsigned long long *host_acc_dev_ = nullptr;
  int ensure_host_buffers();
  int64_t host_chunk_size(int64_t cnt) const;
  int wait_host_flag(int ch, unsigned long long seq);
  RtcKernels rtc_;
  const RtcKernels *rtc() const { return rtc_.module ? &rtc_ : nullptr; }
  void free_later(void *p);
  std::vector<void *> deferred_free_;
  int build_cdf_blocks(const ShardBlocks &rho_blocks, int64_t *len_out, int *any_negative);
  P2PView p2p_view() const;
  int take_silence() {
    if (p2p_skip_ > 0) { --p2p_skip_; return 0; }
    if (p2p_silent_ > 0) { --p2p_silent_; return p2p_loss_ ? 2 : 1; }
    return 0;
  }
  bool p2p_finish();
  void flip_cur() { cur_ = 1 - cur_; ++flips_; if (page_) page_->cur_parity.store((uint32_t)cur_, std::memory_order_relaxed); }
  double *peer_pop_cur(int r) const { return peer_pop_[(peer_cur0_[r] ^ (int)(flips_ & 1u)) & 1][r]; }
  uint32_t tag(uint32_t seq) const { return p2p_tag(gen_, seq); }
  int selftest_patterns(const P2PView &pv);
  bool open_peer_page(int r, const P2PDesc &d);
  uint64_t *slots_ = nullptr;
  uint64_t *peer_slots_[kMaxPeers] = {nullptr};
  double *peer_pop_[2][kMaxPeers] = {{nullptr}};
  double *peer_rho_[kMaxPeers] = {nullptr};
  int peer_cur0_[kMaxPeers] = {0};
  uint32_t flips_ = 0;
  std::vector<void *> ipc_opened_;
  P2PHostPage *page_ = nullptr;
  char page_name_[48] = {0};
  const P2PHostPage *peer_page_[kMaxPeers] = {nullptr};
  bool peer_page_shm_[kMaxPeers] = {false};
  uint32_t gen_ = 0;
  bool mapped_ = false;
  bool exported_ = false;
  double destroy_wait_ms_ = -1.0;
  int p2p_stale_ = 0;
  bool p2p_on_ = false, pending_xchg_ = false;
  uint32_t xseq_ = 0, bseq_ = 0, call_ = 0;
  double p2p_timeout_ms_ = 5000.0;
  int wall_clock_khz_ = 100000;
  int p2p_silent_ = 0, p2p_skip_ = 0;
  bool p2p_loss_ = false;
  double *p2p_test_dev_ = nullptr;
  double *snap_pop_ = nullptr, *snap_rho_ = nullptr;
  int64_t launches_ = 0;
  int64_t persist_max_ = 65536;
  unsigned long long *persist_sync_ = nullptr;
  unsigned long long *persist_rows_ = nullptr;
  int64_t persist_rows_wg_ = 0;
  int persist_lanes_ = 0;
  int prof_ = 0, prof_open_ = -1;
  unsigned prof_tick_ = 0;
  struct EvPair { hipEvent_t a, b; };
  std::vector<EvPair> ev_[SABC_KERNEL_COUNT];
  std::vector<EvPair> ev_pool_;
  double prof_ms_[SABC_KERNEL_COUNT] = {0};
  int64_t prof_n_[SABC_KERNEL_COUNT] = {0};
  int64_t prof_noop_[SABC_KERNEL_COUNT] = {0};
};

}
```

### simulatedannealingabc.jl_amd/csrc/kernels.hip

```cpp
#include <hip/hip_runtime.h>
#include <hip/hip_ext.h>
#include <cstdlib>
#include <cstring>
#ifdef SABC_RC_TIMING
__device__ unsigned long long g_rc_ticks[16];
__device__ __forceinline__ void rc_mark(int i) {
  static __shared__ unsigned long long last;
  if (threadIdx.x != 0) return;
  const unsigned long long t = wall_clock64();
  if (i == 0) atomicAdd(&g_rc_ticks[0], 1ull); else atomicAdd(&g_rc_ticks[i], t - last);
  last = t;
}
#define SABC_CTRL_MARK(i) rc_mark(i)
#endif
#include "control.hpp"
#include "p2p.hpp"
#include "persistent_kernel.hpp"
#include "update_kernel.hpp"

namespace sabc {

constexpr int kGkD = 4, kGkS = 4;
constexpr int kGkPerBlock = (kBlock / 64) * kGkParticlesPerWave;
#ifndef SABC_GK_REPS
// ... 581 lines not shown
}

__device__ __forceinline__ bool p2p_allreduce_rows(const P2PView &pv, const uint32_t seq, const int np, double *mine,
                                                   uint32_t *words, volatile int *failed, const int silent) {
  const int W = pv.world, nw = 2 * np, ring = (int)(seq % kP2PRing);
  const uint32_t *half = reinterpret_cast<const uint32_t *>(mine);
  if (silent != 1)
    for (int i = threadIdx.x; i < W * nw; i += blockDim.x) {
      const int p = i / nw, t = i - p * nw;
      if (silent == 2 && p != pv.rank) continue;
      p2p_store(pv.slots[p] + kP2PSumsOff + ((int64_t)ring * kMaxPeers + pv.rank) * kP2PWords + t, ((uint64_t)seq << 32) | half[t]);
    }
  const uint64_t t0 = p2p_clock();
  for (int i = threadIdx.x; i < W * nw; i += blockDim.x) {
    const int r = i / nw, t = i - r * nw;
    const uint64_t w = p2p_wait_word(pv.slots[pv.rank] + kP2PSumsOff + ((int64_t)ring * kMaxPeers + r) * kP2PWords + t, seq, t0,
                                     pv.timeout_ticks, failed, r, pv.slots[pv.rank]);
    words[i] = (uint32_t)w;
  }
  __syncthreads();
  if (*failed) return false;
  if ((int)threadIdx.x < np) {
    const int q = threadIdx.x;
    double a = 0.0;
    for (int r = 0; r < W; ++r) {
      const double x = __hiloint2double((int)words[r * nw + 2 * q + 1], (int)words[r * nw + 2 * q]);
      a = r == 0 ? x : a + x;
    }
    mine[q] = a;
  }
  __syncthreads();
  return true;
}

struct XchgArgs {
  P2PView pv;
  uint32_t seq;
  int32_t do_control, silent, reserved;
};

template <int CTRL>
__device__ __forceinline__ double dpp_row_shr(double v) {
  const int lo = __builtin_amdgcn_update_dpp(0, __double2loint(v), CTRL, 0xF, 0xF, true);
  const int hi = __builtin_amdgcn_update_dpp(0, __double2hiint(v), CTRL, 0xF, 0xF, true);
  return __hiloint2double(hi, lo);
}

#ifdef SABC_RC_TIMING
#define RC_MARK(i) rc_mark(i)
#else
#define RC_MARK(i) do { } while (0)
#endif

template <bool XCHG>
__global__ void __launch_bounds__(1024)
k_reduce_control(const double *__restrict__ partials, const int64_t rows, const int np, double *__restrict__ stage,
                 ControlBlock *cb, const ControlArgs a, double *hist, Mailbox *ring, const XchgArgs x) {
  __shared__ ControlBlock lcb;
  __shared__ int ran;
  __shared__ int failed;
  __shared__ double sm[1024];
  __shared__ double sums[kMaxPartials];
  __shared__ uint32_t words[XCHG ? kMaxPeers * kP2PWords : 1];
  RC_MARK(0);
  const int B = blockDim.x;
  const int G = B / np;
  const int g = threadIdx.x / np, c = threadIdx.x - g * np;
  constexpr int kInFlight = 24;
  double xx[kInFlight];
  if (rows >= 0 && g < G) {
#pragma unroll
    for (int e = 0; e < kInFlight; ++e) {
      const int64_t r = g + (int64_t)e * G;
      xx[e] = r < rows ? partials[r * np + c] : 0.0;
    }
  }
  control_load(lcb, cb);
#ifdef SABC_RC_TIMING
  __builtin_amdgcn_s_waitcnt(0);
  RC_MARK(7);
#endif
  if (threadIdx.x == 0) failed = 0;
  if (rows >= 0) {
    double v = 0.0;
    if (g < G) {
#pragma unroll
      for (int e = 0; e < kInFlight; ++e) v += xx[e];
      for (int64_t r0 = g + (int64_t)kInFlight * G; r0 < rows; r0 += (int64_t)kInFlight * G) {
#pragma unroll
        for (int e = 0; e < kInFlight; ++e) {
          const int64_t r = r0 + (int64_t)e * G;
          xx[e] = r < rows ? partials[r * np + c] : 0.0;
        }
#pragma unroll
        for (int e = 0; e < kInFlight; ++e) v += xx[e];
      }
    }
    sm[threadIdx.x] = v;
    __syncthreads();
    RC_MARK(1);
    const int n_waves = B >> 6;
    if (np <= 16) {
      const int w = threadIdx.x >> 6, l = threadIdx.x & 63;
      for (int col = w; col < np; col += n_waves) {
        double t = 0.0;
        for (int gg = l; gg < G; gg += 64) t += sm[gg * np + col];
        t += dpp_row_shr<0x111>(t);
        t += dpp_row_shr<0x112>(t);
        t += dpp_row_shr<0x114>(t);
        t += dpp_row_shr<0x118>(t);
// ... 822 lines not shown
}
#endif

int64_t persistent_workgroups_bound(const ModelDesc &m, int64_t cap) {
  if (!persistent_fits(m.d, m.s)) return 0;
  const int64_t A = update_block_threads(m.s) - 64 < 256 ? update_block_threads(m.s) - 64 : 256, wg16 = (16 * cap + A - 1) / A;
  return wg16 < persist_max_workgroups() ? wg16 : persist_max_workgroups();
}

int launch_update_persistent(const ModelDesc &m, int prop_kind, const PersistArgs &pa_in, ControlBlock *cb, PopPtrs pp, CdfPtrs cdf,
                             PartnerView pv_a, PartnerView pv_b, double *partials, double *hist, Mailbox *mbox, double *stage,
                             hipStream_t stream, const RtcKernels *rtc) {
  int lanes = 1, active = 0;
  const int64_t wg = persistent_workgroups(m, prop_kind, pa_in.act_n, rtc, &lanes, &active);
  if (wg <= 0) return (int)hipErrorInvalidValue;
  PersistArgs pa = pa_in;
  pa.active = active;
  pa.ctrl_wave = active < (int)update_block_threads(m.s) ? active / 64 : -1;
  const dim3 grid((unsigned)wg), block((unsigned)update_block_threads(m.s));
  if (m.model_id == SABC_MODEL_USER)
    return module_launch(lanes == 16 ? rtc->persistent16[prop_kind] : lanes == 4 ? rtc->persistent4[prop_kind] : rtc->persistent[prop_kind], grid.x, block.x, stream, nullptr, nullptr, m, pa,
                         cb, pp, cdf, pv_a, pv_b, partials, hist, mbox, stage);
#define PCALLL(M, D, S, P, L) hipLaunchKernelGGL((k_update_persistent<M, D, S, P, L>), grid, block, 0, stream, m, pa, cb, pp, cdf, pv_a, pv_b, partials, hist, mbox, stage)
#define PCALLP(M, D, S, P)                      \
  if (lanes == 16) PCALLL(M, D, S, P, 16);      \
  else if (lanes == 4) PCALLL(M, D, S, P, 4);   \
  else PCALLL(M, D, S, P, 1)
#define PCALL(M, D, S)                                                          \
  switch (prop_kind) {                                                          \
    case SABC_PROP_RANDOMWALK: PCALLP(M, D, S, SABC_PROP_RANDOMWALK); break;     \
    case SABC_PROP_DIFFEVO: PCALLP(M, D, S, SABC_PROP_DIFFEVO); break;           \
    default: PCALLP(M, D, S, SABC_PROP_STRETCH); break;                          \
  }
  if (m.model_id == SABC_MODEL_GAUSS_IID) {
    if (m.d == 1 && m.s == 1) { PCALL(SABC_MODEL_GAUSS_IID, 1, 1); }
    else if (m.d == 1 && m.s == 2) { PCALL(SABC_MODEL_GAUSS_IID, 1, 2); }
    else if (m.d == 2 && m.s == 1) { PCALL(SABC_MODEL_GAUSS_IID, 2, 1); }
    else { PCALL(SABC_MODEL_GAUSS_IID, 2, 2); }
  } else if (m.model_id == SABC_MODEL_GAUSS2D) {
    PCALL(SABC_MODEL_GAUSS2D, 2, 3);
  } else {
    PCALL(SABC_MODEL_LV, 3, 4);
  }
#undef PCALL
#undef PCALLP
#undef PCALLL
  return SABC_LAUNCH_RC();
}

int launch_update(const ModelDesc &m, const StepArgs &c, const ControlBlock *cb, PopPtrs pp, CdfPtrs cdf, PartnerView pv,
                  int64_t act_lo, int64_t act_n, double *partials, int64_t row0, hipStream_t stream, hipEvent_t ev0,
                  hipEvent_t ev1, const RtcKernels *rtc) {
  if (act_n <= 0) return 0;
  const dim3 grid((unsigned)update_rows(m, act_n)), block(m.model_id == SABC_MODEL_GK ? kBlock : update_block_threads(m.s));
  double *out = partials + row0 * n_partials(m.d, m.s);
  if (m.model_id == SABC_MODEL_USER) {
    if (!rtc || c.prop_kind < 0 || c.prop_kind > 2 || !rtc->update[c.prop_kind]) return (int)hipErrorInvalidValue;
    const unsigned b = source_wide(m.s) ? kWideBlock : update_block_threads(m.s);
    return module_launch(rtc->update[c.prop_kind], grid.x, b, stream, ev0, ev1, m, c, cb, pp, cdf, pv, act_lo, act_n, out);
  }
  if (m.model_id == SABC_MODEL_GK) {
    const dim3 g((unsigned)update_rows(m, act_n));
    bool rows4 = SABC_GK_ROWS4 != 0;
    for (int j = 0; j < kGkS; ++j) rows4 = rows4 && (((int)m.p[2 + j]) & 15) == 0 && (int)m.p[2 + j] >= 16 && (int)m.p[2 + j] <= 128;
    switch (c.prop_kind * 2 + (rows4 ? 1 : 0)) {
      case SABC_PROP_RANDOMWALK * 2: SABC_LAUNCH_UPDATE((k_update_gk<SABC_PROP_RANDOMWALK, false>), g); break;
      case SABC_PROP_RANDOMWALK * 2 + 1: SABC_LAUNCH_UPDATE((k_update_gk<SABC_PROP_RANDOMWALK, true>), g); break;
      case SABC_PROP_DIFFEVO * 2: SABC_LAUNCH_UPDATE((k_update_gk<SABC_PROP_DIFFEVO, false>), g); break;
      case SABC_PROP_DIFFEVO * 2 + 1: SABC_LAUNCH_UPDATE((k_update_gk<SABC_PROP_DIFFEVO, true>), g); break;
      case SABC_PROP_STRETCH * 2: SABC_LAUNCH_UPDATE((k_update_gk<SABC_PROP_STRETCH, false>), g); break;
      case SABC_PROP_STRETCH * 2 + 1: SABC_LAUNCH_UPDATE((k_update_gk<SABC_PROP_STRETCH, true>), g); break;
      default: return (int)hipErrorInvalidValue;
    }
    return SABC_LAUNCH_RC();
  }
#define CALLP(M, D, S, P) SABC_LAUNCH_UPDATE((k_update<M, D, S, P>), grid)
#define CALL(M, D, S)                                                           \
  switch (c.prop_kind) {                                                        \
    case SABC_PROP_RANDOMWALK: CALLP(M, D, S, SABC_PROP_RANDOMWALK); break;     \
    case SABC_PROP_DIFFEVO: CALLP(M, D, S, SABC_PROP_DIFFEVO); break;           \
    case SABC_PROP_STRETCH: CALLP(M, D, S, SABC_PROP_STRETCH); break;           \
    default: return (int)hipErrorInvalidValue;                                  \
  }
  SABC_DISPATCH_MODEL(m, CALL);
#undef CALL
#undef CALLP
  return SABC_LAUNCH_RC();
}

int launch_host_prior(const ModelDesc &m, PopPtrs pp, hipStream_t stream) {
  if (pp.n_local <= 0) return 0;
  hipLaunchKernelGGL(k_host_prior, dim3((unsigned)n_blocks(pp.n_local)), dim3(kBlock), 0, stream, m, pp);
  return SABC_LAUNCH_RC();
}

int launch_host_propose(const ModelDesc &m, const StepArgs &c, const ControlBlock *cb, PopPtrs pp, PartnerView pv,
                        int64_t act_lo, int64_t act_n, double *thp, double *aux, double *thp_host, unsigned char *gate_host,
                        double *cur_out, unsigned int *done, unsigned long long *flag, unsigned long long seq, int64_t chunk,
                        hipStream_t stream) {
  if (act_n <= 0) return 0;
  HostSignal sig;
  sig.done = done; sig.flag = flag; sig.seq = seq; sig.chunk = chunk;
  hipLaunchKernelGGL(k_host_propose, dim3((unsigned)n_blocks(act_n)), dim3(kBlock), 0, stream, m, c, cb, pp, pv, act_lo, act_n,
                     thp, aux, thp_host, gate_host, cur_out, sig);
  return SABC_LAUNCH_RC();
}

int launch_host_accept(const ModelDesc &m, const StepArgs &c, const ControlBlock *cb, PopPtrs pp, CdfPtrs cdf, int64_t act_lo,
                       int64_t act_n, int64_t t_lo, int64_t t_n, const double *thp, const double *aux, const double *rho_prop,
                       const double *lp_host, unsigned long long *n_accept, hipStream_t stream) {
  if (t_n <= 0) return 0;
  hipLaunchKernelGGL(k_host_accept, dim3((unsigned)n_blocks(t_n)), dim3(kBlock), 0, stream, m, c, cb, pp, cdf, act_lo, act_n,
                     t_lo, t_n, thp, aux, rho_prop, lp_host, n_accept);
  return SABC_LAUNCH_RC();
}

int launch_stats_rt(const ModelDesc &m, const ControlBlock *cb, PopPtrs pp, double *partials, unsigned long long *n_accept,
                    hipStream_t stream) {
  if (pp.n_local <= 0) return 0;
  hipLaunchKernelGGL(k_stats_rt, dim3((unsigned)n_blocks(pp.n_local)), dim3(kBlock), 0, stream, m.d, m.s, cb, pp, partials,
                     n_accept);
  return SABC_LAUNCH_RC();
}

int launch_stats(const ModelDesc &m, const ControlBlock *cb, PopPtrs pp, double *partials, hipStream_t stream,
                 const RtcKernels *rtc) {
  if (pp.n_local <= 0) return 0;
  if (m.model_id == SABC_MODEL_HOST) return launch_stats_rt(m, cb, pp, partials, nullptr, stream);
  if (m.model_id == SABC_MODEL_USER) {
    if (!rtc || !rtc->stats) return (int)hipErrorInvalidValue;
    return module_launch(rtc->stats, (unsigned)n_blocks(pp.n_local), kBlock, stream, nullptr, nullptr, cb, pp, partials);
  }
  const dim3 grid((unsigned)n_blocks(pp.n_local)), block(kBlock);
#define CALL(M, D, S) hipLaunchKernelGGL((k_stats<D, S>), grid, block, 0, stream, cb, pp, partials)
  if (m.model_id == SABC_MODEL_GK) { CALL(SABC_MODEL_GK, 4, 4); return SABC_LAUNCH_RC(); }
  SABC_DISPATCH_MODEL(m, CALL);
#undef CALL
  return SABC_LAUNCH_RC();
}

int launch_reduce_partials(const double *partials, int64_t rows, int np, double *sums, const int *halt,
                           hipStream_t stream) {
  hipLaunchKernelGGL(k_reduce_partials, dim3((unsigned)np), dim3(kBlock), 0, stream, partials, rows, np, sums, halt);
  return SABC_LAUNCH_RC();
}

int launch_reduce_control(const double *partials, int64_t rows, int np, double *stage, bool reduce_guarded,
                          ControlBlock *cb, const ControlArgs &a, double *hist, Mailbox *mbox, hipStream_t stream,
                          const P2PView *pv, uint32_t seq, bool do_control, int silent) {
  (void)reduce_guarded;
  XchgArgs x;
  std::memset(&x, 0, sizeof(x));
  x.do_control = do_control ? 1 : 0;
  static const int forced = [] { const char *e = std::getenv("SABC_RC_BLOCK"); const int v = e ? std::atoi(e) : 0; return (v == 256 || v == 1024) ? v : 0; }();
  const int block = forced && np <= 256 ? forced : ((rows < 0 && np <= 256) || (np <= 64 && rows >= 0 && rows <= (int64_t)24 * (256 / np))) ? 256 : 1024;
  if (pv) {
    x.pv = *pv; x.seq = seq; x.silent = silent;
    hipLaunchKernelGGL(k_reduce_control<true>, dim3(1), dim3(block), 0, stream, partials, rows, np, stage, cb, a, hist, mbox, x);
  } else {
    hipLaunchKernelGGL(k_reduce_control<false>, dim3(1), dim3(block), 0, stream, partials, rows, np, stage, cb, a, hist, mbox, x);
  }
  return SABC_LAUNCH_RC();
}

int launch_p2p_barrier(const P2PView &pv, uint32_t seq, ControlBlock *cb, bool guarded, int silent, hipStream_t stream) {
  hipLaunchKernelGGL(k_p2p_barrier, dim3(1), dim3(64), 0, stream, pv, seq, cb, guarded ? 1 : 0, silent);
  return SABC_LAUNCH_RC();
}

int launch_p2p_commit(const P2PView &pv, uint32_t call, int status, bool wait, ControlBlock *cb, int silent, hipStream_t stream) {
  hipLaunchKernelGGL(k_p2p_commit, dim3(1), dim3(64), 0, stream, pv, call, status, wait ? 1 : 0, cb, silent);
  return SABC_LAUNCH_RC();
}

int launch_p2p_selftest(const P2PView &pv, uint32_t seq, int np, const double *in, double *out, int *failed, int silent,
                        hipStream_t stream) {
  hipLaunchKernelGGL(k_p2p_selftest, dim3(1), dim3(1024), 0, stream, pv, seq, np, in, out, failed, silent);
  return SABC_LAUNCH_RC();
}

int launch_p2p_leave(const P2PView &pv, uint32_t gen, hipStream_t stream) {
  hipLaunchKernelGGL(k_p2p_leave, dim3(1), dim3(64), 0, stream, pv, gen);
  return SABC_LAUNCH_RC();
}

static PatternBufs pattern_bufs(double *const buf[3], const int64_t len[3]) {
  PatternBufs g;
  for (int b = 0; b < 3; ++b) {
    g.buf[b] = reinterpret_cast<uint64_t *>(buf[b]);
    g.len[b] = len[b];
    g.count[b] = (int32_t)(len[b] < kPatternSamples ? len[b] : kPatternSamples);
  }
  return g;
}
int p2p_pattern_save_words() { return 3 * kPatternSamples; }
int launch_p2p_pattern_write(double *const buf[3], const int64_t len[3], double *save, uint32_t gen, int round, int rank, int mode,
                             hipStream_t stream) {
  hipLaunchKernelGGL(k_p2p_pattern_write, dim3(kPatternSamples / 256, 3), dim3(256), 0, stream, pattern_bufs(buf, len),
                     reinterpret_cast<uint64_t *>(save), gen, round, rank, mode);
  return SABC_LAUNCH_RC();
}
int launch_p2p_pattern_check(const double *const peer_buf[3][kMaxPeers], const int64_t len[3], uint32_t gen, int round, int world,
                             unsigned int *out, hipStream_t stream) {
  PatternPeers pp;
  for (int b = 0; b < 3; ++b)
    for (int r = 0; r < kMaxPeers; ++r) pp.buf[b][r] = reinterpret_cast<const uint64_t *>(peer_buf[b][r]);
  double *none[3] = {nullptr, nullptr, nullptr};
  hipLaunchKernelGGL(k_p2p_pattern_check, dim3(kPatternSamples / 256, 3, world), dim3(256), 0, stream, pp, pattern_bufs(none, len), gen,
                     round, world, out);
  return SABC_LAUNCH_RC();
}

int launch_control(ControlBlock *cb, const ControlArgs &a, double *hist, Mailbox *mbox, const double *sums_in,
// ... 227 lines not shown
```

### simulatedannealingabc.jl_amd/csrc/kernels.hpp

```cpp
#pragma once
#include "sabc_types.hpp"
#include "p2p.hpp"
#if !defined(__HIPCC_RTC__)
#include <hip/hip_runtime_api.h>
#include "rtc.hpp"
#endif

namespace sabc {

struct PopPtrs {
  double *pop;
  double *rho;
  int64_t cap, n_local, gid0;
};

#ifndef SABC_CDF_COARSE
#define SABC_CDF_COARSE 1024
#endif
#ifndef SABC_CDF_COARSE_MS
#define SABC_CDF_COARSE_MS 2048
#endif
#ifndef SABC_UPDATE_BLOCK_MS
#define SABC_UPDATE_BLOCK_MS 512
#endif
// ... 14 lines not shown
constexpr int kBlock = 256;
#ifndef SABC_UPDATE_BLOCK
#define SABC_UPDATE_BLOCK 256
#endif
constexpr int update_block_threads(int s) { return s <= 1 ? SABC_UPDATE_BLOCK : SABC_UPDATE_BLOCK_MS; }
#ifndef SABC_UPDATE_MIN_WAVES
#define SABC_UPDATE_MIN_WAVES 4
#endif
#ifndef SABC_UPDATE_MIN_WAVES_MS
#define SABC_UPDATE_MIN_WAVES_MS 6
#endif
constexpr int update_min_waves(int s) {
  return s <= 1 ? SABC_UPDATE_MIN_WAVES : 3 * (cdf_coarse_entries(s) * s * 8 + 4096) <= 160 * 1024 ? SABC_UPDATE_MIN_WAVES_MS : SABC_UPDATE_MIN_WAVES;
}
constexpr bool update_loop_trimmed(int model, int d, int s, int prop, bool one_launch) {
  if (one_launch) return model != 2 && model != 4;
  if (model == 2 && prop != 0) return false;
  if (model == 1 && d == 2 && s == 2 && prop == 1) return false;
  return true;
}
constexpr int update_loop_coop(int model, int d, int s, int prop, bool one_launch) {
  return update_loop_trimmed(model, d, s, prop, one_launch) ? 0 : -1;
}
constexpr int kNarrowStats = 16;
constexpr int kWideBlock = 64;
constexpr bool source_wide(int s) { return s > kNarrowStats; }
constexpr int kScanChunk = 1024;
#ifndef SABC_FUSE_REDUCE_MAX
#define SABC_FUSE_REDUCE_MAX 32768
#endif
constexpr int64_t kFuseReduceMaxDoubles = SABC_FUSE_REDUCE_MAX;

inline int64_t n_blocks(int64_t n) { return (n + kBlock - 1) / kBlock; }

struct PersistArgs {
  uint64_t iter0;
  int64_t ix0, phase, cph;
  int64_t act_n, half;
  int32_t count;
  int32_t test_absent_wg;
  int32_t active;
  int32_t ctrl_wave;
  double prop_p0, prop_p1;
  ControlArgs ctrl;
  unsigned long long *sync;
  uint64_t timeout_ticks;
  uint64_t rendezvous_ticks;
};
constexpr bool persistent_fits(int d, int s) {
  return !source_wide(s) && (long)s * cdf_coarse_entries(s) * 8 + 3072 + (long)(update_block_threads(s) / 64 + 2) * n_partials(d, s) * 8 +
         (long)update_block_threads(s) * 8 + (long)sizeof(ControlBlock) + (long)kMaxPartials * 8 + 2048 <= 156 * 1024;
}

#if !defined(__HIPCC_RTC__)
int launch_prior_simulate(const ModelDesc &m, PopPtrs pp, hipStream_t stream, const RtcKernels *rtc = nullptr);
int launch_cdf_population(const ModelDesc &m, PopPtrs pp, CdfPtrs cdf, hipStream_t stream);
int launch_update(const ModelDesc &m, const StepArgs &c, const ControlBlock *cb, PopPtrs pp, CdfPtrs cdf, PartnerView pv,
                  int64_t act_lo, int64_t act_n, double *partials, int64_t row0, hipStream_t stream,
                  hipEvent_t ev0 = nullptr, hipEvent_t ev1 = nullptr, const RtcKernels *rtc = nullptr);
int64_t persistent_workgroups(const ModelDesc &m, int prop_kind, int64_t act_n, const RtcKernels *rtc = nullptr, int *lanes_out = nullptr,
                              int *active_out = nullptr);
int64_t persistent_workgroups_bound(const ModelDesc &m, int64_t cap);
int launch_update_persistent(const ModelDesc &m, int prop_kind, const PersistArgs &pa, ControlBlock *cb, PopPtrs pp, CdfPtrs cdf,
                             PartnerView pv_a, PartnerView pv_b, double *partials, double *hist, Mailbox *mbox, double *stage,
                             hipStream_t stream, const RtcKernels *rtc = nullptr);
int64_t update_rows(const ModelDesc &m, int64_t act_n);
int launch_stats(const ModelDesc &m, const ControlBlock *cb, PopPtrs pp, double *partials, hipStream_t stream,
                 const RtcKernels *rtc = nullptr);
int launch_reduce_partials(const double *partials, int64_t rows, int np, double *sums, const int *halt,
                           hipStream_t stream);
int launch_control(ControlBlock *cb, const ControlArgs &a, double *hist, Mailbox *mbox, const double *sums_in,
                   hipStream_t stream);
int launch_reduce_control(const double *partials, int64_t rows, int np, double *stage, bool reduce_guarded,
                          ControlBlock *cb, const ControlArgs &a, double *hist, Mailbox *mbox, hipStream_t stream,
                          const P2PView *pv = nullptr, uint32_t seq = 0, bool do_control = true, int silent = 0);
int launch_p2p_barrier(const P2PView &pv, uint32_t seq, ControlBlock *cb, bool guarded, int silent, hipStream_t stream);
int launch_p2p_commit(const P2PView &pv, uint32_t call, int status, bool wait, ControlBlock *cb, int silent, hipStream_t stream);
int launch_p2p_selftest(const P2PView &pv, uint32_t seq, int np, const double *in, double *out, int *failed, int silent,
                        hipStream_t stream);
int launch_p2p_leave(const P2PView &pv, uint32_t gen, hipStream_t stream);
int p2p_pattern_save_words();
int launch_p2p_pattern_write(double *const buf[3], const int64_t len[3], double *save, uint32_t gen, int round, int rank, int mode,
                             hipStream_t stream);
int launch_p2p_pattern_check(const double *const peer_buf[3][kMaxPeers], const int64_t len[3], uint32_t gen, int round, int world,
                             unsigned int *out, hipStream_t stream);
int launch_resample_weights(const ModelDesc &m, PopPtrs pp, const ControlBlock *cb, double n_global, double delta,
                            hipStream_t stream);
inline int64_t weight_scan_doubles(int64_t n_global) {
  const int64_t nb = (n_global + kScanChunk - 1) / kScanChunk;
  return 2 * nb + nb * (kScanChunk / 16);
}
int launch_weight_scan(const ShardBlocks &gathered, int64_t n_global, double *block_sums,
                       double *cum, double *totals, double *totals_host, hipStream_t stream);
int launch_resample_local(const ModelDesc &m, PopPtrs src, PopPtrs dst, const ControlBlock *cb, double delta, uint64_t iter,
                          double *block_sums, double *cum, double *totals, double *totals_host, double *pack,
                          double *partials, int64_t *stats_rows, hipStream_t stream);
int64_t resample_pack_doubles(int row_len, int64_t n);
int launch_resample_gather(const ModelDesc &m, const ShardBlocks &gathered, int64_t n_global,
                           const double *cum, const double *block_sums, const double *totals, uint64_t iter, PopPtrs dst,
                           hipStream_t stream);
int launch_resample_select(const ModelDesc &m, int64_t cap, int64_t n_global, const double *cum, const double *block_sums,
                           const double *totals, uint64_t iter, PopPtrs dst, int64_t *idx_out, hipStream_t stream);
int launch_bucket_count(const int64_t *idx, int64_t n_local, int64_t cap, unsigned long long *counts, hipStream_t stream);
int launch_bucket_scatter(const int64_t *idx, int64_t n_local, int64_t cap, unsigned long long *cursor, double *req,
                          int64_t *slot, hipStream_t stream);
int launch_resample_serve(const double *req, int64_t m, int row_len, PopPtrs src, double *rows_out, hipStream_t stream);
int launch_resample_scatter(const double *rows_in, const int64_t *slot, int64_t n_local, int row_len, PopPtrs dst,
                            hipStream_t stream);
int launch_cdf_knots(const double *sorted, int64_t n, double *knots, int64_t *meta, hipStream_t stream);
int launch_cdf_index(double *knots, int64_t len, int64_t stride, int shift, double *coarse, int n_coarse, double *mid,
                     int64_t mid_len, hipStream_t stream);
int launch_compact_column(const ShardBlocks &gathered, int stat, int64_t n_global, double *out, hipStream_t stream);
int sort_f64(const double *in, double *out, int64_t n, void *tmp, size_t *tmp_bytes, hipStream_t stream);
int launch_host_prior(const ModelDesc &m, PopPtrs pp, hipStream_t stream);
int launch_host_propose(const ModelDesc &m, const StepArgs &c, const ControlBlock *cb, PopPtrs pp, PartnerView pv,
                        int64_t act_lo, int64_t act_n, double *thp, double *aux, double *thp_host, unsigned char *gate_host,
                        double *cur_out, unsigned int *done, unsigned long long *flag, unsigned long long seq, int64_t chunk,
                        hipStream_t stream);
int launch_host_accept(const ModelDesc &m, const StepArgs &c, const ControlBlock *cb, PopPtrs pp, CdfPtrs cdf, int64_t act_lo,
                       int64_t act_n, int64_t t_lo, int64_t t_n, const double *thp, const double *aux, const double *rho_prop,
                       const double *lp_host, unsigned long long *n_accept, hipStream_t stream);
int launch_stats_rt(const ModelDesc &m, const ControlBlock *cb, PopPtrs pp, double *partials, unsigned long long *n_accept,
                    hipStream_t stream);
int launch_cdf_eval(const double *knots, int64_t len, const double *q, int64_t m, double *out, hipStream_t stream);
int launch_cdf_apply_matrix(CdfPtrs cdf, int s, const double *rho, int64_t m, double *u_out, hipStream_t stream);
int launch_simulate_batch(const ModelDesc &m, const double *theta, int64_t n, uint64_t pid0, uint64_t iter,
                          double *rho_out, hipStream_t stream, const RtcKernels *rtc = nullptr, const unsigned char *gate = nullptr);
int launch_prior_op(const ModelDesc &m, uint64_t pid0, int64_t n, double *theta, double *lp, hipStream_t stream,
// ... 11 lines not shown
```

### simulatedannealingabc.jl_amd/csrc/rtc.cpp

```cpp
#include "rtc.hpp"

#include <dlfcn.h>
#include <sys/stat.h>
#include <unistd.h>

#include <cstdio>
#include <cstdlib>
#include <cstring>
#include <map>
#include <mutex>
#include <vector>

#include "../../include/sabc_hip.h"
#include "kernels.hpp"

namespace sabc {

namespace {

struct HiprtcApi {
  void *lib = nullptr;
  int (*CreateProgram)(void **, const char *, const char *, int, const char **, const char **) = nullptr;
  int (*DestroyProgram)(void **) = nullptr;
  int (*CompileProgram)(void *, int, const char **) = nullptr;
// ... 127 lines not shown
  const std::string t = path + tmp;
  FILE *fp = std::fopen(t.c_str(), "wb");
  if (!fp) return;
  const uint64_t head[3] = {kDiskMagic, (uint64_t)n_kernels, (uint64_t)m.code.size()};
  bool ok = std::fwrite(head, sizeof(head), 1, fp) == 1;
  for (int i = 0; ok && i < n_kernels; ++i) {
    const uint32_t len = (uint32_t)m.lowered[i].size();
    ok = std::fwrite(&len, sizeof(len), 1, fp) == 1 && std::fwrite(m.lowered[i].data(), 1, len, fp) == len;
  }
  ok = ok && std::fwrite(m.code.data(), 1, m.code.size(), fp) == m.code.size();
  const uint64_t tail = kDiskMagic ^ head[2];
  ok = ok && std::fwrite(&tail, sizeof(tail), 1, fp) == 1;
  ok = (std::fclose(fp) == 0) && ok;
  if (ok) ok = std::rename(t.c_str(), path.c_str()) == 0;
  if (!ok) (void)std::remove(t.c_str());
}

}

std::string rtc_default_csrc_dir() {
  Dl_info info;
  if (dladdr((void *)&anchor, &info) && info.dli_fname) {
    std::string p(info.dli_fname);
    const size_t slash = p.rfind('/');
    return (slash == std::string::npos ? std::string(".") : p.substr(0, slash)) + "/csrc";
  }
  return "csrc";
}

void rtc_release(RtcKernels *k) {
  if (k && k->module) (void)hipModuleUnload(k->module);
  if (k) *k = RtcKernels();
}

int rtc_build(const char *user_source, int d, int s, const std::string &csrc_dir, RtcKernels *out, std::string *log,
              bool user_prior, bool with_persistent) {
  return rtc_compile(user_source, d, s, csrc_dir, out, log, nullptr, user_prior, with_persistent);
}

int rtc_compile(const char *user_source, int d, int s, const std::string &csrc_dir, RtcKernels *out, std::string *log,
                size_t *code_size, bool user_prior, bool with_persistent) {
  constexpr int kMaxKernels = 16;
  const bool wide = source_wide(s);
  if (wide) with_persistent = false;
  const int kKernels = with_persistent ? 16 : 7;
  HiprtcApi *api = hiprtc_api();
  if (!api) { *log = "libhiprtc.so could not be loaded: simulators from source need the hipRTC of ROCm"; return -1; }
  if (d < 1 || d > SABC_MAX_PARA || s < 1 || s > SABC_MAX_SOURCE_STATS) { *log = "n_para / n_stats out of range (a simulator from source: d <= 16, s <= 64)"; return -1; }
  char tail[2048];
  std::snprintf(tail, sizeof(tail),
                "\nnamespace sabc {\n"
                "template <int D, int S>\n"
                "struct Sim<SABC_MODEL_USER, D, S> {\n"
                "  static __device__ __forceinline__ void run(const ModelDesc &m, const double *th, uint64_t pid, uint64_t iter,\n"
                "                                             double *rho, int coop = 0) {\n"
                "    NormalStream ns(m.seed, pid, PURPOSE_SIM, iter, coop);\n"
                "    ::sabc_user_simulate(th, m.p, ns, rho);\n"
                "  }\n"
                "};\n"
                "}  // namespace sabc\n");
  std::string src = std::string("#include \"update_kernel.hpp\"\n") + (with_persistent ? "#include \"persistent_kernel.hpp\"\n" : "") + "#line 1 \"f_dist.hip\"\n";
  src += user_source;
  src += tail;

  char name[kMaxKernels][112];
  const char *w = wide ? "_wide" : "";
  std::snprintf(name[0], sizeof(name[0]), "sabc::k_prior_simulate%s<%d, %d, %d>", w, SABC_MODEL_USER, d, s);
  for (int p = 0; p < 3; ++p) std::snprintf(name[1 + p], sizeof(name[1 + p]), "sabc::k_update%s<%d, %d, %d, %d>", w, SABC_MODEL_USER, d, s, p);
  std::snprintf(name[4], sizeof(name[4]), "sabc::k_simulate_batch%s<%d, %d, %d>", w, SABC_MODEL_USER, d, s);
  std::snprintf(name[5], sizeof(name[5]), "sabc::k_stats%s<%d, %d>", w, d, s);
  std::snprintf(name[6], sizeof(name[6]), "sabc::k_prior_op_t<%d>", d);
  for (int p = 0; p < 3; ++p) std::snprintf(name[7 + p], sizeof(name[7 + p]), "sabc::k_update_persistent<%d, %d, %d, %d>", SABC_MODEL_USER, d, s, p);
  for (int p = 0; p < 3; ++p) std::snprintf(name[10 + p], sizeof(name[10 + p]), "sabc::k_update_persistent<%d, %d, %d, %d, 4>", SABC_MODEL_USER, d, s, p);
  for (int p = 0; p < 3; ++p) std::snprintf(name[13 + p], sizeof(name[13 + p]), "sabc::k_update_persistent<%d, %d, %d, %d, 16>", SABC_MODEL_USER, d, s, p);
  const char *extra_env = std::getenv("SABC_RTC_EXTRA_FLAGS");
  const std::string extra = extra_env ? extra_env : "";

#define SABC_RTC_STR2(x) #x
#define SABC_RTC_STR(x) SABC_RTC_STR2(x)
  static const char *geometry = SABC_RTC_STR(SABC_UPDATE_BLOCK) "," SABC_RTC_STR(SABC_UPDATE_BLOCK_MS) "," SABC_RTC_STR(SABC_CDF_COARSE) ","
                                SABC_RTC_STR(SABC_CDF_COARSE_MS) "," SABC_RTC_STR(SABC_UPDATE_MIN_WAVES) "," SABC_RTC_STR(SABC_UPDATE_MIN_WAVES_MS);
#undef SABC_RTC_STR
#undef SABC_RTC_STR2
  const std::string cache_key = std::to_string(d) + "," + std::to_string(s) + (user_prior ? ",P" : "") + (with_persistent ? ",1L4L16" : "") + "," + extra + "," +
                                geometry + "\n" + user_source;
  if (out) {
    std::lock_guard<std::mutex> lock(g_cache_mutex);
    auto hit = g_cache.find(cache_key);
    if (hit != g_cache.end()) {
      RtcKernels k;
      k.d = d; k.s = s;
      if (hipModuleLoadData(&k.module, hit->second.code.data()) != hipSuccess) { *log = "hipModuleLoadData of the cached simulator failed"; return -1; }
      hipFunction_t *slots[kMaxKernels] = {&k.prior_simulate, &k.update[0], &k.update[1], &k.update[2], &k.simulate_batch, &k.stats, &k.prior_op,
                                        &k.persistent[0], &k.persistent[1], &k.persistent[2], &k.persistent4[0], &k.persistent4[1], &k.persistent4[2],
                                        &k.persistent16[0], &k.persistent16[1], &k.persistent16[2]};
      for (int i = 0; i < kKernels; ++i)
        if (hipModuleGetFunction(slots[i], k.module, hit->second.lowered[i].c_str()) != hipSuccess) {
          *log = std::string("kernel not found in the cached module: ") + name[i];
          rtc_release(&k);
          return -1;
        }
      if (code_size) *code_size = hit->second.code.size();
      *out = k;
      return 0;
    }
  }
// ... 118 lines not shown
```

### simulatedannealingabc.jl_amd/csrc/sabc_types.hpp

```cpp
#pragma once
#include <stdint.h>
#include "../../include/sabc_hip.h"

#if defined(__HIPCC__)
#define SABC_TYPES_HD __host__ __device__
#else
#define SABC_TYPES_HD
#endif

namespace sabc {

constexpr int kMaxPara = SABC_MAX_PARA;
constexpr int kMaxStats = SABC_MAX_STATS;
constexpr int kMaxJointPara = SABC_MAX_JOINT_PARA;

struct ModelDesc {
  int32_t model_id, d, s, n_model_params;
  double p[SABC_MAX_MODEL_PARAMS];
  int32_t prior_kind[kMaxPara];
  double prior_a[kMaxPara], prior_b[kMaxPara], prior_c[kMaxPara], prior_d[kMaxPara];
  double prior_logc[kMaxPara];
  double prior_k0[kMaxPara], prior_k1[kMaxPara];
  int32_t prior_joint, prior_pad;
  double prior_L[kMaxJointPara * kMaxJointPara];
  double prior_joint_logc;
  uint64_t seed;
};

struct StepArgs {
  uint64_t iter;
  int32_t prop_kind, reserved;
  double prop_p0, prop_p1;
};

struct ControlBlock {
  double eps[kMaxStats];
  double beta[kMaxStats];
  double chol[kMaxPara * kMaxPara];
  double sigma[kMaxPara * kMaxPara];
  double pivot[kMaxPara];
  double sums[1 + 2 * kMaxStats + kMaxPara + kMaxPara * (kMaxPara + 1) / 2];
  int64_t n_accept;
  int64_t hist_rows;
  int64_t persist_done;
  int32_t error;
  int32_t eps_len;
  int32_t halt;
  int32_t comm_where;
};

enum : int32_t {
  CTRL_ACCUMULATE = 1,
  CTRL_PROPOSAL = 2,
  CTRL_EPSILON = 4,
  CTRL_PIVOT = 8,
  CTRL_HISTORY = 16,
  CTRL_CHECK = 32,
  CTRL_CLEAR_HALT = 64,
  CTRL_GUARDED = 128,
  CTRL_KEEP_SUMS = 256
};

struct ControlArgs {
  int32_t mode, d, s, algorithm, prop_kind;
  int32_t rho_is_delta;
  double n_global, v, prop_p0;
  int64_t hist_capacity;
  int64_t notify_seq;
  double resample_threshold;
};

struct Mailbox {
  volatile uint64_t w0, w1;
};
inline constexpr uint64_t kMailboxEmpty = ~0ull;
SABC_TYPES_HD inline void mailbox_pack(int64_t seq, int64_t n_accept, int32_t error, int32_t halted, uint64_t *w0, uint64_t *w1) {
  const uint64_t s32 = (uint64_t)(uint32_t)seq << 32, na = (uint64_t)n_accept;
  *w0 = s32 | (na & 0xFFFFFFFFull);
  *w1 = s32 | ((uint64_t)(halted ? 1 : 0) << 31) | ((uint64_t)((uint32_t)(-error) & 0xFFu) << 23) | ((na >> 32) & 0x7FFFFFull);
}
SABC_TYPES_HD inline bool mailbox_unpack(uint64_t w0, uint64_t w1, int64_t seq, int64_t *n_accept, int32_t *error, int32_t *halted) {
  const uint32_t s32 = (uint32_t)seq;
  if ((uint32_t)(w0 >> 32) != s32 || (uint32_t)(w1 >> 32) != s32) return false;
  *n_accept = (int64_t)((w0 & 0xFFFFFFFFull) | ((w1 & 0x7FFFFFull) << 32));
  *error = -(int32_t)((w1 >> 23) & 0xFFu);
// ... 58 lines not shown
```

### simulatedannealingabc.jl_amd/csrc/update_kernel.hpp

```cpp
#pragma once
#include "device_models.hpp"
#include "kernels.hpp"

namespace sabc {

template <int NP, int BLOCK = kBlock, int FIRST = 1>
__device__ __forceinline__ void block_reduce_store(const double (&acc)[NP], double *__restrict__ out) {
  constexpr int NW = BLOCK / 64;
  __shared__ double sm[NW][NP];
  const int lane = threadIdx.x & 63, wave = threadIdx.x >> 6;
  double v[NP];
#pragma unroll
  for (int c = 0; c < NP; ++c) v[c] = acc[c];
#pragma unroll
  for (int off = 32; off >= FIRST; off >>= 1) {
    double t[NP];
#pragma unroll
    for (int c = 0; c < NP; ++c) t[c] = __shfl_down(v[c], off, 64);
#pragma unroll
    for (int c = 0; c < NP; ++c) v[c] += t[c];
  }
  if (lane == 0) {
#pragma unroll
    for (int c = 0; c < NP; ++c) sm[wave][c] = v[c];
// ... 31 lines not shown
  r = (int64_t)((double)gid / (double)cap);
  if (r * cap > gid) r -= 1;
  else if ((r + 1) * cap <= gid) r += 1;
  o = gid - r * cap;
}

__device__ __forceinline__ const double *partner_ptr(const PartnerView &pv, uint64_t j) {
  if (pv.world == 1) return pv.base + pv.off_last + (int64_t)j;
  int64_t r = (int64_t)((double)j / (double)pv.m_full);
  if (r * pv.m_full > (int64_t)j) r -= 1;
  else if ((r + 1) * pv.m_full <= (int64_t)j) r += 1;
  if (r > pv.world - 1) r = pv.world - 1;
  const int64_t o = (int64_t)j - r * pv.m_full;
  const int64_t off = (r == pv.world - 1) ? pv.off_last : pv.off_full;
  const double *b = pv.direct ? pv.peer[r] : pv.base + r * pv.rank_stride;
  return b + off + o;
}

__device__ __forceinline__ const double *shard_block(const ShardBlocks &b, int64_t r) {
  return b.direct ? b.peer[r] : b.flat + r * (int64_t)b.rows * b.cap;
}

template <int S>
__device__ __forceinline__ void load_coarse_index(const CdfPtrs &cdf, double (&cidx)[S][cdf_coarse_entries(S)]) {
  constexpr int kUpdateBlock = update_block_threads(S), kCoarse = cdf_coarse_entries(S);
  static_assert((S * kCoarse / 2) % kUpdateBlock == 0, "whole passes of 16 bytes per thread");
  constexpr int kPasses = S * kCoarse / 2 / kUpdateBlock;
  const double2 *src = reinterpret_cast<const double2 *>(cdf.coarse);
  double2 *dst = reinterpret_cast<double2 *>(&cidx[0][0]);
  double2 tmp[kPasses];
#pragma unroll
  for (int q = 0; q < kPasses; ++q) tmp[q] = src[threadIdx.x + q * kUpdateBlock];
#pragma unroll
  for (int q = 0; q < kPasses; ++q) dst[threadIdx.x + q * kUpdateBlock] = tmp[q];
}

#ifdef SABC_PERSIST_TRACE
__device__ unsigned long long g_persist_trace[64 * 16];
#define SABC_TRACE(iter, i) do { if (blockIdx.x == 0 && threadIdx.x == 0) g_persist_trace[((iter) & 63) * 16 + (i)] = (unsigned long long)wall_clock64(); } while (0)
#else
#define SABC_TRACE(iter, i) do { } while (0)
#endif

template <bool PAST_CACHES>
__device__ __forceinline__ double particle_load(const double *p) {
  return PAST_CACHES ? __hip_atomic_load(p, __ATOMIC_RELAXED, __HIP_MEMORY_SCOPE_AGENT) : *p;
}
template <bool PAST_CACHES>
__device__ __forceinline__ void particle_store(double *p, double v) {
  if (PAST_CACHES) __hip_atomic_store(p, v, __ATOMIC_RELAXED, __HIP_MEMORY_SCOPE_AGENT);
  else *p = v;
}

template <int D, int S>
struct ParticleDraft {
  double th[D], u[S];
  double thp[D], rp[S];
  double logf, lpp;
};

template <int MODEL, int D, int S, int PROP, bool PAST_CACHES, int LANES, bool ONE_LAUNCH = false, class CB>
__device__ __forceinline__ void update_particle_draft(const ModelDesc &m, const uint64_t iter, const double prop_p0, const double prop_p1,
                                                      const CB *__restrict__ cb, const PopPtrs &pp, const PartnerView &pv, const int64_t li,
                                                      const uint64_t gid, ParticleDraft<D, S> &q) {
#pragma unroll
  for (int k = 0; k < D; ++k) q.th[k] = pp.pop[(int64_t)k * pp.cap + li];
#pragma unroll
  for (int j = 0; j < S; ++j) q.u[j] = pp.pop[(int64_t)(D + j) * pp.cap + li];

  SABC_TRACE(iter, 6);
  q.logf = 0.0;
  if (PROP == SABC_PROP_RANDOMWALK) {
    NormalStream ns(m.seed, gid, PURPOSE_PROP, iter, LANES > 1 ? LANES : 0);
    double z[D];
#pragma unroll
    for (int k = 0; k < D; ++k) z[k] = ns.next();
#pragma unroll
    for (int k = 0; k < D; ++k) {
      double a = 0.0;
#pragma unroll
      for (int l = 0; l <= k; ++l) a += cb->chol[k * D + l] * z[l];
      q.thp[k] = q.th[k] + a;
    }
  } else if (PROP == SABC_PROP_DIFFEVO) {
    uint64_t i1 = 0, i2 = 0;
    for (uint32_t a = 0;; ++a) {
      const u32x4 w = stream_block(m.seed, gid, PURPOSE_PROP, iter, a);
      i1 = mulhi64(pack64(w.x, w.y), (uint64_t)pv.m_total);
      i2 = mulhi64(pack64(w.z, w.w), (uint64_t)pv.m_total);
      if (i1 != i2 || a > 64u) break;
    }
    double z0, z1;
    box_muller(stream_block(m.seed, gid, PURPOSE_PROP2, iter, 0), z0, z1);
    const double gamma = prop_p0 * (1.0 + prop_p1 * z0);
    const double *p1 = partner_ptr(pv, i1), *p2 = partner_ptr(pv, i2);
#pragma unroll
    for (int k = 0; k < D; ++k)
      q.thp[k] = q.th[k] + gamma * (particle_load<PAST_CACHES>(p1 + (int64_t)k * pv.cap) - particle_load<PAST_CACHES>(p2 + (int64_t)k * pv.cap));
  } else {
    const u32x4 w = stream_block(m.seed, gid, PURPOSE_PROP, iter, 0);
    const uint64_t ip = mulhi64(pack64(w.x, w.y), (uint64_t)pv.m_total);
    const double U = u52(w.z, w.w);
    const double a = prop_p0;
    const double tt = (a - 1.0) * U + 1.0;
    const double z = tt * tt / a;
    const double *p = partner_ptr(pv, ip);
#pragma unroll
    for (int k = 0; k < D; ++k) {
      const double pk = particle_load<PAST_CACHES>(p + (int64_t)k * pv.cap);
      q.thp[k] = pk + z * (q.th[k] - pk);
    }
    q.logf = log(z) * (double)(D - 1);
  }

  SABC_TRACE(iter, 7);
  q.lpp = prior_logpdf<D>(m, q.thp);
#pragma unroll
  for (int j = 0; j < S; ++j) q.rp[j] = 0.0;
  if (q.lpp > -INFINITY) {
    if (LANES > 1) Sim<MODEL, D, S>::run(m, q.thp, gid, iter, q.rp, LANES);
    else Sim<MODEL, D, S>::run(m, q.thp, gid, iter, q.rp, update_loop_coop(MODEL, D, S, PROP, ONE_LAUNCH));
  }
  SABC_TRACE(iter, 8);
}

template <int D, int S, bool PAST_CACHES, int LANES, bool LATENCY, class CB>
__device__ __forceinline__ void update_particle_decide(const ModelDesc &m, const uint64_t iter, const CB *__restrict__ cb, const PopPtrs &pp,
                                                       const CdfPtrs &cdf, const double (&cidx)[S][cdf_coarse_entries(S)], const int64_t li,
                                                       const uint64_t gid, ParticleDraft<D, S> &q, double (&acc)[n_partials(D, S)]) {
  constexpr int kCoarse = cdf_coarse_entries(S);
  double log_accept = -INFINITY;
  double up[S], drho[S];
#pragma unroll
  for (int j = 0; j < S; ++j) { up[j] = 0.0; drho[j] = 0.0; }
  if (q.lpp > -INFINITY) {
    double a = 0.0;
    if (LATENCY && S >= 2) cdf_apply_3level_lockstep<S, kCoarse>(cdf, cidx, q.rp, up);
#pragma unroll
    for (int j = 0; j < S; ++j) {
      if (LATENCY && S == 1 && cdf.shift[0] == 0)
        up[j] = cdf_apply_lds<kCoarse>(cidx[j], cdf.len[j], q.rp[j]);
      else if (!(LATENCY && S >= 2))
        up[j] = cdf_apply_3level<kCoarse>(cdf.knots + (int64_t)j * cdf.stride, cdf.len[j], cdf.shift[j], cidx[j],
                                 cdf.mid + (int64_t)j * cdf.mid_stride, q.rp[j]);
      const double e = (cb->eps_len == 1) ? cb->eps[0] : cb->eps[j];
      a += (q.u[j] - up[j]) / e;
    }
    log_accept = q.lpp - prior_logpdf<D>(m, q.th) + a + q.logf;
  }

  SABC_TRACE(iter, 9);
  const u32x4 wa = stream_block(m.seed, gid, PURPOSE_ACCEPT, iter, 0);
  const bool accepted = -0.5 * neg2_log_tab(u52(wa.x, wa.y)) < log_accept;
  const bool writer = LANES == 1 || (threadIdx.x & (LANES - 1)) == 0;
  if (accepted) {
#pragma unroll
    for (int j = 0; j < S; ++j) drho[j] = q.rp[j] - pp.rho[(int64_t)j * pp.cap + li];
#pragma unroll
    for (int k = 0; k < D; ++k) q.th[k] = q.thp[k];
#pragma unroll
    for (int j = 0; j < S; ++j) q.u[j] = up[j];
    if (writer) {
#pragma unroll
      for (int k = 0; k < D; ++k) particle_store<PAST_CACHES>(pp.pop + (int64_t)k * pp.cap + li, q.thp[k]);
#pragma unroll
      for (int j = 0; j < S; ++j) {
        pp.pop[(int64_t)(D + j) * pp.cap + li] = up[j];
        pp.rho[(int64_t)j * pp.cap + li] = q.rp[j];
      }
    }
  }
  SABC_TRACE(iter, 10);
  moment_terms<D, S>(cb->pivot, accepted, q.th, q.u, drho, acc);
  if (!writer) {
#pragma unroll
    for (int q2 = 0; q2 < n_partials(D, S); ++q2) acc[q2] = 0.0;
  }
}

template <int MODEL, int D, int S, int PROP, bool PAST_CACHES = false, int LANES = 1, bool LATENCY = false, class CB>
__device__ __forceinline__ void update_particle(const ModelDesc &m, const uint64_t iter, const double prop_p0, const double prop_p1,
                                                const CB *__restrict__ cb, const PopPtrs &pp, const CdfPtrs &cdf, const PartnerView &pv,
                                                const double (&cidx)[S][cdf_coarse_entries(S)], const int64_t li, const uint64_t gid,
                                                double (&acc)[n_partials(D, S)]) {
  ParticleDraft<D, S> q;
  update_particle_draft<MODEL, D, S, PROP, PAST_CACHES, LANES, LATENCY>(m, iter, prop_p0, prop_p1, cb, pp, pv, li, gid, q);
  update_particle_decide<D, S, PAST_CACHES, LANES, LATENCY>(m, iter, cb, pp, cdf, cidx, li, gid, q, acc);
}

template <int MODEL, int D, int S, int PROP>
__global__ void __launch_bounds__(update_block_threads(S), update_min_waves(S))
k_update(const ModelDesc m, const StepArgs c, const ControlBlock *__restrict__ cb, const PopPtrs pp, const CdfPtrs cdf,
         const PartnerView pv, const int64_t act_lo, const int64_t act_n, double *__restrict__ partials) {
  constexpr int NP = n_partials(D, S);
  if (cb->halt) return;
  rng_tables_load();
  constexpr int kUpdateBlock = update_block_threads(S), kCoarse = cdf_coarse_entries(S);
  __shared__ double cidx[S][kCoarse];
  load_coarse_index<S>(cdf, cidx);
  __syncthreads();
  double acc[NP];
#pragma unroll
  for (int q = 0; q < NP; ++q) acc[q] = 0.0;

  const int64_t t = (int64_t)blockIdx.x * kUpdateBlock + threadIdx.x;
  if (t < act_n) {
    const int64_t li = act_lo + t;
    update_particle<MODEL, D, S, PROP>(m, c.iter, c.prop_p0, c.prop_p1, cb, pp, cdf, pv, cidx, li, (uint64_t)(pp.gid0 + li), acc);
  }
  block_reduce_store<NP, kUpdateBlock>(acc, partials + (int64_t)blockIdx.x * NP);
}

template <int D, int S>
__global__ void __launch_bounds__(kBlock)
k_stats(const ControlBlock *__restrict__ cb, const PopPtrs pp, double *__restrict__ partials) {
  constexpr int NP = n_partials(D, S);
  double acc[NP];
#pragma unroll
  for (int q = 0; q < NP; ++q) acc[q] = 0.0;
  const int64_t li = (int64_t)blockIdx.x * kBlock + threadIdx.x;
  if (li < pp.n_local) {
    double th[D], u[S], rho[S];
#pragma unroll
    for (int k = 0; k < D; ++k) th[k] = pp.pop[(int64_t)k * pp.cap + li];
#pragma unroll
    for (int j = 0; j < S; ++j) {
      u[j] = pp.pop[(int64_t)(D + j) * pp.cap + li];
      rho[j] = pp.rho[(int64_t)j * pp.cap + li];
    }
    moment_terms<D, S>(cb->pivot, false, th, u, rho, acc);
  }
  block_reduce_store<NP>(acc, partials + (int64_t)blockIdx.x * NP);
}

template <int MODEL, int D, int S>
__global__ void __launch_bounds__(kBlock) k_prior_simulate(const ModelDesc m, const PopPtrs pp) {
  rng_tables_init();
  const int64_t li = (int64_t)blockIdx.x * kBlock + threadIdx.x;
  if (li >= pp.n_local) return;
  const uint64_t gid = (uint64_t)(pp.gid0 + li);
  double th[D], rho[S];
  prior_sample<D>(m, gid, th);
  Sim<MODEL, D, S>::run(m, th, gid, 0, rho);
#pragma unroll
  for (int k = 0; k < D; ++k) pp.pop[(int64_t)k * pp.cap + li] = th[k];
#pragma unroll
  for (int j = 0; j < S; ++j) pp.rho[(int64_t)j * pp.cap + li] = rho[j];
}

template <int D>
__global__ void __launch_bounds__(kBlock)
k_prior_op_t(const ModelDesc m, const uint64_t pid0, const int64_t n, double *__restrict__ theta, double *__restrict__ lp) {
  rng_tables_init();
  const int64_t i = (int64_t)blockIdx.x * kBlock + threadIdx.x;
  if (i >= n) return;
  double th[D];
  prior_sample<D>(m, pid0 + (uint64_t)i, th);
#pragma unroll
  for (int k = 0; k < D; ++k) theta[(int64_t)k * n + i] = th[k];
  lp[i] = prior_logpdf<D>(m, th);
}

template <int MODEL, int D, int S>
__global__ void __launch_bounds__(kBlock)
k_simulate_batch(const ModelDesc m, const double *__restrict__ theta, const int64_t n, const uint64_t pid0,
                 const uint64_t iter, double *__restrict__ rho_out, const unsigned char *__restrict__ gate) {
  rng_tables_init();
  const int64_t i = (int64_t)blockIdx.x * kBlock + threadIdx.x;
  if (i >= n) return;
  double th[D], rho[S];
#pragma unroll
  for (int j = 0; j < S; ++j) rho[j] = 0.0;
  if (!gate || gate[i]) {
#pragma unroll
    for (int k = 0; k < D; ++k) th[k] = theta[(int64_t)k * n + i];
    Sim<MODEL, D, S>::run(m, th, pid0 + (uint64_t)i, iter, rho);
  }
#pragma unroll
  for (int j = 0; j < S; ++j) rho_out[(int64_t)j * n + i] = rho[j];
}

template <int S>
constexpr int wide_row() { return S | 1; }

constexpr int kDraftOnly = -1;
template <int D, int S>
struct Sim<kDraftOnly, D, S> {
  static __device__ __forceinline__ void run(const ModelDesc &, const double *, uint64_t, uint64_t, double *, int = 0) {}
};

template <int J>
struct StatIdx { static constexpr int value = J; };
template <int J, int N, class F>
__device__ __forceinline__ void static_for(F &f) {
  if constexpr (J < N) {
    f(StatIdx<J>());
    static_for<J + 1, N>(f);
  }
}

__device__ __forceinline__ void column_to_lds(double v, const int c, double *sm, const int np) {
#pragma unroll
  for (int off = 32; off >= 1; off >>= 1) v += __shfl_down(v, off, 64);
  if ((threadIdx.x & 63) == 0) sm[(threadIdx.x >> 6) * np + c] = v;
}

template <int NW>
__device__ __forceinline__ void columns_store(const double *sm, const int np, double *__restrict__ out) {
  __syncthreads();
  for (int c = threadIdx.x; c < np; c += NW * 64) {
    double a = sm[c];
#pragma unroll
    for (int w = 1; w < NW; ++w) a += sm[w * np + c];
    out[c] = a;
  }
}

template <int D>
__device__ __forceinline__ void theta_columns(const double *__restrict__ pivot, const double (&th)[D], const bool live, const int c0,
                                              double *sm, const int np) {
  double dk[D];
#pragma unroll
  for (int k = 0; k < D; ++k) dk[k] = live ? th[k] - pivot[k] : 0.0;
#pragma unroll
  for (int k = 0; k < D; ++k) column_to_lds(dk[k], c0 + k, sm, np);
  int q = c0 + D;
#pragma unroll
  for (int k = 0; k < D; ++k)
#pragma unroll
    for (int l = 0; l <= k; ++l) column_to_lds(dk[k] * dk[l], q++, sm, np);
}

template <int MODEL, int D, int S, int PROP>
__global__ void __launch_bounds__(kWideBlock)
k_update_wide(const ModelDesc m, const StepArgs c, const ControlBlock *__restrict__ cb, const PopPtrs pp, const CdfPtrs cdf,
              const PartnerView pv, const int64_t act_lo, const int64_t act_n, double *__restrict__ partials) {
  constexpr int NP = n_partials(D, S), NW = kWideBlock / 64, R = wide_row<S>(), kCoarse = cdf_coarse_entries(S);
  if (cb->halt) return;
  rng_tables_load();
  __shared__ double rows[kWideBlock * R];
// ... 119 lines not shown
```

### simulatedannealingabc.jl_amd/handle.py

```python
from __future__ import annotations

import ctypes as C

import numpy as np

from . import _lib
from ._lib import Config, SABCError, UpdateArgs


def _dp(a):
    return None if a is None else a.ctypes.data_as(C.POINTER(C.c_double))


class SabcHandle:
    def __init__(self, *, n_particles, model, prior, algorithm=_lib.ALG_SINGLE_EPS, v=1.0, delta=0.1,
                 seed=20241220, device=0, rank=0, world=1):
        cfg = Config()
        cfg.abi_version = _lib.ABI_VERSION
        cfg.device = int(device)
        cfg.n_particles = int(n_particles)
        cfg.n_para = len(prior)
        cfg.n_stats = int(model.n_stats)
        cfg.model_id = int(model.model_id)
        params = list(model.params)
# ... 236 lines not shown
        return out

    def set_cdf_knots(self, stat, knots):
        k = np.ascontiguousarray(knots, dtype=np.float64)
        self._check(self._L.sabc_set_cdf_knots(self._h, stat, _dp(k), len(k)))

    def cdf_apply(self, rho):
        r = np.ascontiguousarray(rho, dtype=np.float64).reshape(self.s, -1)
        out = np.empty_like(r)
        self._check(self._L.sabc_cdf_apply(self._h, _dp(r), r.shape[1], _dp(out)))
        return out

    @property
    def proposal_sigma(self):
        out = np.zeros((self.d, self.d))
        self._check(self._L.sabc_get_proposal_sigma(self._h, _dp(out)))
        return out

    @property
    def ess(self):
        return float(self._L.sabc_last_ess(self._h))

    def simulate(self, theta, pid0, it):
        th = np.ascontiguousarray(theta, dtype=np.float64).reshape(self.d, -1)
        out = np.empty((self.s, th.shape[1]))
        self._check(self._L.sabc_op_simulate(self._h, _dp(th), th.shape[1], int(pid0), int(it), _dp(out)))
        return out

    def prior(self, pid0, m):
        th, lp = np.empty((self.d, int(m))), np.empty(int(m))
        self._check(self._L.sabc_op_prior(self._h, int(pid0), int(m), _dp(th), _dp(lp)))
        return th, lp

    @property
    def host_syncs(self):
        return int(self._L.sabc_host_syncs(self._h))

    def set_host_chunk(self, particles):
        self._check(self._L.sabc_set_host_chunk(self._h, int(particles)))

    @property
    def host_callback_seconds(self):
        return float(self._L.sabc_host_callback_seconds(self._h))

    @property
    def host_callback_calls(self):
        return int(self._L.sabc_host_callback_calls(self._h))

    @property
    def kernel_launches(self):
        return int(self._L.sabc_kernel_launches(self._h))

    @property
    def collective_calls(self):
        return int(self._L.sabc_collective_calls(self._h))

    @property
    def persistent_launches(self):
        fn = getattr(self._L, "sabc_persistent_launches", None)
        return int(fn(self._h)) if fn is not None else 0

    @property
    def persistent_lanes(self):
        return int(self._L.sabc_persistent_lanes(self._h))

    @property
    def persistent_fallbacks(self):
        return int(self._L.sabc_persistent_fallbacks(self._h))

    def profile_enable(self, on=True):
        self._check(self._L.sabc_profile_enable(self._h, int(on)))

    def profile_noops(self, kernel):
        return int(self._L.sabc_profile_noops(self._h, int(kernel)))

    def profile_get(self, kernel):
        ms, cnt = C.c_double(), C.c_int64()
        self._check(self._L.sabc_profile_get(self._h, int(kernel), C.byref(ms), C.byref(cnt)))
        return ms.value, cnt.value


def op_build_cdf(x, device=0):
    x = np.ascontiguousarray(x, dtype=np.float64)
    out = np.zeros(len(x) + 2)
    ln = C.c_int64()
    rc = _lib.lib().sabc_op_build_cdf(device, _dp(x), len(x), _dp(out), C.byref(ln))
    if rc:
        raise SABCError(rc, _lib.global_error())
    return out[: ln.value].copy()


def op_sort(x, device=0):
    x = np.ascontiguousarray(x, dtype=np.float64)
    out = np.empty_like(x)
    rc = _lib.lib().sabc_op_sort(device, _dp(x), len(x), _dp(out))
    if rc:
        raise SABCError(rc, _lib.global_error())
    return out


def op_cdf_eval(knots, q, device=0):
    k = np.ascontiguousarray(knots, dtype=np.float64)
    qq = np.atleast_1d(np.ascontiguousarray(q, dtype=np.float64))
    out = np.empty_like(qq)
    rc = _lib.lib().sabc_op_cdf_eval(device, _dp(k), len(k), _dp(qq), len(qq), _dp(out))
    if rc:
# ... 51 lines not shown
```

Measured before the change: 6.568 billion.

## Precompute next-iteration simulation RNG sums in idle update and reduce slots

Splits the Gaussian model simulators into a draw phase and a finish phase. The draw phase depends only on seed, particle id and iteration, not on theta. Extra producer workgroups appended to the update kernel, plus producer work in the reduce/control kernel, compute the normal-draw sums for the next iteration ahead of time and tag each block. The consumer update kernel looks up these tags and continues drawing from the stored offset rather than from zero. The aim is to fill tail-wave idle CUs and the serial control phase with useful RNG work, at the cost of extra double-buffered sum storage, tag bookkeeping, and a more complex fill heuristic.

```diff
diff --git a/include/sabc_hip.h b/include/sabc_hip.h
--- a/include/sabc_hip.h
+++ b/include/sabc_hip.h
@@ -191,6 +191,7 @@
 SABC_API int64_t sabc_profile_noops(sabc_handle *h, int32_t kernel);
 SABC_API int64_t sabc_host_syncs(const sabc_handle *h);
 SABC_API int64_t sabc_kernel_launches(const sabc_handle *h);
+SABC_API int64_t sabc_ahead_blocks(sabc_handle *h, int32_t which);
 SABC_API int64_t sabc_persistent_launches(const sabc_handle *h);
 SABC_API int32_t sabc_persistent_lanes(const sabc_handle *h);
 SABC_API int64_t sabc_persistent_fallbacks(const sabc_handle *h);
diff --git a/simulatedannealingabc.jl_amd/_lib.py b/simulatedannealingabc.jl_amd/_lib.py
--- a/simulatedannealingabc.jl_amd/_lib.py
+++ b/simulatedannealingabc.jl_amd/_lib.py
@@ -176,6 +176,7 @@
         "sabc_host_callback_calls": ([vp], C.c_int64),
         "sabc_host_syncs": ([vp], C.c_int64),
         "sabc_kernel_launches": ([vp], C.c_int64),
+        "sabc_ahead_blocks": ([vp, C.c_int32], C.c_int64),
         "sabc_persistent_launches": ([vp], C.c_int64),
         "sabc_persistent_lanes": ([vp], C.c_int32),
         "sabc_persistent_fallbacks": ([vp], C.c_int64),
diff --git a/simulatedannealingabc.jl_amd/csrc/capi.hip b/simulatedannealingabc.jl_amd/csrc/capi.hip
--- a/simulatedannealingabc.jl_amd/csrc/capi.hip
+++ b/simulatedannealingabc.jl_amd/csrc/capi.hip
@@ -698,6 +698,7 @@
 
 int64_t sabc_host_syncs(const sabc_handle *h) { return h ? h->eng->host_syncs() : 0; }
 int64_t sabc_kernel_launches(const sabc_handle *h) { return h ? h->be->kernel_launches() : 0; }
+int64_t sabc_ahead_blocks(sabc_handle *h, int32_t which) { return h ? h->be->ahead_blocks(which) : 0; }
 int64_t sabc_collective_calls(const sabc_handle *h) { return h ? h->eng->collective_calls() : 0; }
 
 int sabc_profile_enable(sabc_handle *h, int32_t on) {
diff --git a/simulatedannealingabc.jl_amd/csrc/device_models.hpp b/simulatedannealingabc.jl_amd/csrc/device_models.hpp
--- a/simulatedannealingabc.jl_amd/csrc/device_models.hpp
+++ b/simulatedannealingabc.jl_amd/csrc/device_models.hpp
@@ -378,40 +378,66 @@
 
 template <int D, int S>
 struct Sim<SABC_MODEL_GAUSS_IID, D, S> {
-  static __device__ __forceinline__ void run(const ModelDesc &m, const double *th, uint64_t pid, uint64_t iter,
-                                             double *rho, int coop = 0) {
-    const int n_obs = (int)m.p[0];
-    const double mu = th[0];
-    const double sd = (D >= 2) ? th[1] : m.p[1];
-    NormalStream ns(m.seed, pid, PURPOSE_SIM, iter, coop);
-    double sz = 0.0, szz = 0.0;
-    const int n_pairs = n_obs >> 1;
+  static constexpr int kAheadSums = S >= 2 ? 2 : 1;
+  static __device__ __forceinline__ int loop_pairs(const ModelDesc &m) { return (int)m.p[0] >> 1; }
+  static __device__ __forceinline__ void draw(uint64_t seed, uint64_t pid, uint64_t iter, int first_pair, int n_pairs,
+                                              double (&sums)[kAheadSums], int coop = 0) {
+    NormalStream ns(seed, pid, PURPOSE_SIM, iter, coop);
+    ns.seek((uint32_t)first_pair);
+    double sz = sums[0], szz = S >= 2 ? sums[kAheadSums - 1] : 0.0;
     ns.for_pairs(n_pairs, [&](const double z0, const double z1) {
       sz += z0; if (S >= 2) szz = fma(z0, z0, szz);
       sz += z1; if (S >= 2) szz = fma(z1, z1, szz);
     });
+    sums[0] = sz;
+    if (S >= 2) sums[kAheadSums - 1] = szz;
+  }
+  static __device__ __forceinline__ void finish(const ModelDesc &m, const double *th, uint64_t pid, uint64_t iter,
+                                                const double (&sums)[kAheadSums], double *rho, int coop = 0) {
+    const int n_obs = (int)m.p[0];
+    const double mu = th[0];
+    const double sd = (D >= 2) ? th[1] : m.p[1];
+    double sz = sums[0], szz = S >= 2 ? sums[kAheadSums - 1] : 0.0;
     if (n_obs & 1) {
+      NormalStream ns(m.seed, pid, PURPOSE_SIM, iter, coop);
+      ns.seek((uint32_t)(n_obs >> 1));
       double z0, z1;
       ns.pair(z0, z1);
       sz += z0; if (S >= 2) szz = fma(z0, z0, szz);
     }
     const double n = (double)n_obs;
     rho[0] = fabs(m.p[2] - (mu + sd * sz / n));
-    if (S >= 2) rho[1] = fabs(m.p[3] - (mu * mu + (2.0 * mu * sd * sz + sd * sd * szz) / n));
+    if (S >= 2) rho[1] = fabs(m.p[3] - (mu * mu + fma(2.0 * mu * sd, sz, sd * sd * szz) / n));
+  }
+  static __device__ __forceinline__ void run(const ModelDesc &m, const double *th, uint64_t pid, uint64_t iter,
+                                             double *rho, int coop = 0) {
+    double sums[kAheadSums];
+#pragma unroll
+    for (int q = 0; q < kAheadSums; ++q) sums[q] = 0.0;
+    draw(m.seed, pid, iter, 0, loop_pairs(m), sums, coop);
+    finish(m, th, pid, iter, sums, rho, coop);
   }
 };
 
 template <int D, int S>
 struct Sim<SABC_MODEL_GAUSS2D, D, S> {
-  static __device__ __forceinline__ void run(const ModelDesc &m, const double *th, uint64_t pid, uint64_t iter,
-                                             double *rho, int coop = 0) {
+  static constexpr int kAheadSums = 5;
+  static __device__ __forceinline__ int loop_pairs(const ModelDesc &m) { return (int)m.p[0]; }
+  static __device__ __forceinline__ void draw(uint64_t seed, uint64_t pid, uint64_t iter, int first_pair, int n_pairs,
+                                              double (&sums)[kAheadSums], int coop = 0) {
+    NormalStream ns(seed, pid, PURPOSE_SIM, iter, coop);
+    ns.seek((uint32_t)first_pair);
+    double A = sums[0], B = sums[1], AA = sums[2], BB = sums[3], AB = sums[4];
+    ns.for_pairs(n_pairs, [&](const double za, const double zb) {
+      A += za; B += zb; AA = fma(za, za, AA); BB = fma(zb, zb, BB); AB = fma(za, zb, AB);
+    });
+    sums[0] = A; sums[1] = B; sums[2] = AA; sums[3] = BB; sums[4] = AB;
+  }
+  static __device__ __forceinline__ void finish(const ModelDesc &m, const double *th, uint64_t, uint64_t,
+                                                const double (&sums)[kAheadSums], double *rho, int = 0) {
     const int n_obs = (int)m.p[0];
     const double r = m.p[1], c = sqrt(1.0 - r * r);
-    NormalStream ns(m.seed, pid, PURPOSE_SIM, iter, coop);
-    double A = 0, B = 0, AA = 0, BB = 0, AB = 0;
-    ns.for_pairs(n_obs, [&](const double za, const double zb) {
-      A += za; B += zb; AA = fma(za, za, AA); BB = fma(zb, zb, BB); AB = fma(za, zb, AB);
-    });
+    const double A = sums[0], B = sums[1], AA = sums[2], BB = sums[3], AB = sums[4];
     const double S1 = A, S2 = r * A + c * B;
     const double Q11 = AA, Q22 = r * r * AA + 2.0 * r * c * AB + c * c * BB, Q12 = r * AA + c * AB;
     const double m1 = S1 / n_obs, m2 = S2 / n_obs;
@@ -421,6 +447,14 @@
     rho[0] = sqrt(d1 * d1 + d2 * d2);
     if (S >= 2) rho[1] = fabs(var1 + var2 - m.p[4]);
     if (S >= 3) rho[2] = fabs(cov - m.p[5]);
+  }
+  static __device__ __forceinline__ void run(const ModelDesc &m, const double *th, uint64_t pid, uint64_t iter,
+                                             double *rho, int coop = 0) {
+    double sums[kAheadSums];
+#pragma unroll
+    for (int q = 0; q < kAheadSums; ++q) sums[q] = 0.0;
+    draw(m.seed, pid, iter, 0, loop_pairs(m), sums, coop);
+    finish(m, th, pid, iter, sums, rho, coop);
   }
 };
 
@@ -698,6 +732,7 @@
 
 template <int D, int S>
 struct Sim<SABC_MODEL_LV, D, S> {
+  static constexpr int kAheadSums = 0;
   static __device__ __forceinline__ void run(const ModelDesc &m, const double *th, uint64_t pid, uint64_t iter,
                                              double *rho, int coop = 0) {
     const int n_steps = (int)m.p[0];
diff --git a/simulatedannealingabc.jl_amd/csrc/device_rng.hpp b/simulatedannealingabc.jl_amd/csrc/device_rng.hpp
--- a/simulatedannealingabc.jl_amd/csrc/device_rng.hpp
+++ b/simulatedannealingabc.jl_amd/csrc/device_rng.hpp
@@ -336,6 +336,7 @@
   __device__ __forceinline__ NormalStream(uint64_t seed_, uint64_t pid_, uint32_t purpose_, uint64_t iter_, int coop_ = 0)
       : seed(seed_), pid(pid_), iter(iter_), purpose(purpose_), k(0), spare(0.0), have(false), coop(coop_), buf_block(-1),
         buf_uniform(false), b0(0.0), b1(0.0) {}
+  __device__ __forceinline__ void seek(uint32_t block) { k = block; have = false; }
   __device__ __forceinline__ void pair(double &z0, double &z1) {
     if (coop == 4) { fetch<4>(k++, false, z0, z1); return; }
     if (coop == 16) { fetch<16>(k++, false, z0, z1); return; }
diff --git a/simulatedannealingabc.jl_amd/csrc/hip_backend.hip b/simulatedannealingabc.jl_amd/csrc/hip_backend.hip
--- a/simulatedannealingabc.jl_amd/csrc/hip_backend.hip
+++ b/simulatedannealingabc.jl_amd/csrc/hip_backend.hip
@@ -74,6 +74,83 @@
     const long long v = std::atoll(e);
     if (v >= 0) fuse_reduce_max_ = v;
   }
+  if (const char *e = std::getenv("SABC_AHEAD_A")) ahead_a_ = std::atoll(e) < 0 ? -1 : std::atoll(e);
+  if (const char *e = std::getenv("SABC_AHEAD_PAIRS")) ahead_pairs_ = std::atoll(e) < 0 ? -1 : std::atoll(e);
+  if (const char *e = std::getenv("SABC_AHEAD_FILL")) ahead_fill_ = (e[0] == 'a' || std::atoll(e) < 0) ? -1 : std::atoll(e);
+}
+
+int HipBackend::ahead_alloc() {
+  const char *e = std::getenv("SABC_AHEAD");
+  const int ns = ahead_sums_per_particle(m_.model_id, m_.s);
+  if ((e && e[0] == '0') || ns == 0 || sh_.world != 1 || sh_.cap <= 0) return 0;
+  int cus = 0;
+  if (hipDeviceGetAttribute(&cus, hipDeviceAttributeMultiprocessorCount, device_) == hipSuccess && cus > 0) cu_count_ = cus;
+  else (void)hipGetLastError();
+  ahead_n_blocks_ = (sh_.cap + kAheadBlock - 1) / kAheadBlock;
+  ahead_tag_words_ = ahead_n_blocks_ + 4;
+  const size_t sums_bytes = (size_t)ns * (size_t)sh_.cap * sizeof(double), tag_bytes = (size_t)(2 * ahead_tag_words_ + 2) * sizeof(unsigned long long);
+  for (int q = 0; q < 2; ++q) HB_CHECK(hipMalloc((void **)&ahead_sums_[q], sums_bytes), "hipMalloc(ahead sums)");
+  HB_CHECK(hipMalloc((void **)&ahead_tags_[0], tag_bytes), "hipMalloc(ahead tags)");
+  ahead_tags_[1] = ahead_tags_[0] + ahead_tag_words_;
+  ahead_counts_ = ahead_tags_[1] + ahead_tag_words_;
+  HB_CHECK(hipMemsetAsync(ahead_tags_[0], 0, tag_bytes, stream_), "hipMemset(ahead tags)");
+  return 0;
+}
+
+int HipBackend::ahead_clear() {
+  ahead_step_pending_ = false;
+  ahead_covered_[0] = ahead_covered_[1] = 0;
+  if (!ahead_tags_[0]) return 0;
+  HB_CHECK(hipMemsetAsync(ahead_tags_[0], 0, (size_t)(2 * ahead_tag_words_) * sizeof(unsigned long long), stream_), "hipMemset(ahead tags)");
+  return 0;
+}
+
+int64_t HipBackend::ahead_blocks(int which) {
+  if (!ahead_counts_ || which < 0 || which > 1) return 0;
+  unsigned long long v[2] = {0, 0};
+  if (hipMemcpyAsync(v, ahead_counts_, sizeof(v), hipMemcpyDeviceToHost, stream_) != hipSuccess || hipStreamSynchronize(stream_) != hipSuccess) {
+    (void)hipGetLastError();
+    return -1;
+  }
+  return (int64_t)v[which];
+}
+
+bool HipBackend::ahead_update_args(const StepArgs &c, int64_t lo, int64_t cnt, int64_t rows, AheadArgs *out) {
+  std::memset(out, 0, sizeof(*out));
+  ahead_step_pending_ = false;
+  if (!ahead_tags_[0] || c.prop_kind != SABC_PROP_RANDOMWALK || lo != 0 || cnt != sh_.n_local || cnt <= 0) return false;
+  const int64_t nb = (sh_.n_local + kAheadBlock - 1) / kAheadBlock;
+  const int64_t total_pairs = m_.model_id == SABC_MODEL_GAUSS2D ? (int64_t)m_.p[0] : ((int64_t)m_.p[0] >> 1);
+  int64_t pairs = ahead_pairs_ < 0 || ahead_pairs_ > total_pairs ? total_pairs : ahead_pairs_;
+  if (pairs >= ((int64_t)1 << kAheadPairBits)) pairs = ((int64_t)1 << kAheadPairBits) - 1;
+  for (int q = 0; q < 2; ++q) { out->sums[q] = ahead_sums_[q]; out->tags[q] = ahead_tags_[q]; }
+  out->counts = ahead_counts_;
+  out->own_blocks = (int32_t)rows;
+  out->prod_pairs = (int32_t)pairs;
+  int64_t a = ahead_a_ < 0 ? cu_count_ - 1 : ahead_a_;
+  if (a > nb) a = nb;
+  if (pairs <= 0) a = 0;
+  const int64_t per_wg = update_block_threads(m_.s) / kAheadBlock;
+  int64_t f = ahead_fill_;
+  if (f < 0) {
+    constexpr double kRest = 0.15;
+    const double loop_share = (1.0 - kRest) * (double)pairs / (double)(total_pairs > 0 ? total_pairs : 1);
+    const int64_t covered = ahead_covered_iter_[c.iter & 1] == c.iter ? ahead_covered_[c.iter & 1] : 0;
+    const double work = ((double)nb - loop_share * (double)covered) / (double)per_wg;
+    const double rounds = std::ceil(work / (double)cu_count_ - 1e-9);
+    f = (int64_t)((rounds * (double)cu_count_ - work) * (double)per_wg / (loop_share > 0 ? loop_share : 1.0));
+  }
+  if (f > nb - a) f = nb - a;
+  if (f < 0 || pairs <= 0 || !update_carries_producers(m_.model_id, m_.s)) f = 0;
+  out->prod_block0 = (int32_t)a;
+  out->prod_blocks = (int32_t)f;
+  ahead_step_pending_ = true;
+  ahead_step_iter_ = c.iter;
+  ahead_step_blocks_ = a;
+  ahead_step_pairs_ = pairs;
+  ahead_covered_[(c.iter + 1) & 1] = a + f;
+  ahead_covered_iter_[(c.iter + 1) & 1] = c.iter + 1;
+  return true;
 }
 
 void HipBackend::free_later(void *p) {
@@ -125,6 +202,9 @@
   rtc_release(&rtc_);
   if (persist_sync_) (void)hipFree(persist_sync_);
   if (persist_rows_) (void)hipFree(persist_rows_);
+  for (double *p : ahead_sums_)
+    if (p) (void)hipFree(p);
+  if (ahead_tags_[0]) (void)hipFree(ahead_tags_[0]);
   if (slots_) (void)hipFree(slots_);
   if (p2p_test_dev_) (void)hipFree(p2p_test_dev_);
   if (snap_pop_) (void)hipFree(snap_pop_);
@@ -226,6 +306,7 @@
   HB_CHECK(hipMalloc((void **)&totals_dev_, 2 * sizeof(double)), "hipMalloc(totals)");
   totals_host_[0] = totals_host_[1] = 0.0;
   HB_CHECK(hipMalloc((void **)&meta_dev_, 2 * kMaxStats * sizeof(int64_t)), "hipMalloc(meta)");
+  if (ahead_alloc()) return -1;
   int khz = 0;
   if (hipDeviceGetAttribute(&khz, hipDeviceAttributeWallClockRate, device_) == hipSuccess && khz > 0) wall_clock_khz_ = khz;
   else (void)hipGetLastError();
@@ -548,6 +629,7 @@
 
 int HipBackend::prior_simulate() {
   if (m_.model_id == SABC_MODEL_USER && !rtc()) { err_ = "no device simulator registered (sabc_register_device_simulator)"; return -1; }
+  if (ahead_clear()) return -1;
   prof_begin(SABC_KERNEL_INIT);
   HB_LAUNCH(launch_prior_simulate(m_, pop_ptrs(cur_), stream_, rtc()), "k_prior_simulate");
   prof_end(SABC_KERNEL_INIT);
@@ -611,7 +693,9 @@
     else if (hipEventCreate(&e.a) != hipSuccess || hipEventCreate(&e.b) != hipSuccess) e = EvPair{nullptr, nullptr};
     if (e.a && e.b) { ev_[SABC_KERNEL_UPDATE].push_back(e); ev0 = e.a; ev1 = e.b; }
   }
-  HB_LAUNCH(launch_update(m_, c, cb_dev_, pop_ptrs(cur_), cdf_ptrs(), pv, lo, cnt, partials_, row0, stream_, ev0, ev1, rtc()), "k_update");
+  StepArgs ca = c;
+  (void)ahead_update_args(c, lo, cnt, rows, &ca.ahead);
+  HB_LAUNCH(launch_update(m_, ca, cb_dev_, pop_ptrs(cur_), cdf_ptrs(), pv, lo, cnt, partials_, row0, stream_, ev0, ev1, rtc()), "k_update");
   *rows_out = rows;
   return 0;
 }
@@ -662,6 +746,7 @@
 }
 
 int HipBackend::stats(int64_t *rows_out) {
+  ahead_step_pending_ = false;
   HB_LAUNCH(launch_stats(m_, cb_dev_, pop_ptrs(cur_), partials_, stream_, rtc()), "k_stats");
   *rows_out = n_blocks(sh_.n_local);
   return 0;
@@ -702,13 +787,26 @@
 int HipBackend::control(const ControlArgs &a) {
   const bool xchg = pending_xchg_ && pending_rows_ >= 0;
   const P2PView pv = xchg ? p2p_view() : P2PView();
+  AheadProd ap;
+  std::memset(&ap, 0, sizeof(ap));
+  if (ahead_step_pending_ && pending_rows_ >= 0 && !xchg && ahead_step_blocks_ > 0) {
+    for (int q = 0; q < 2; ++q) { ap.ah.sums[q] = ahead_sums_[q]; ap.ah.tags[q] = ahead_tags_[q]; }
+    ap.ah.counts = ahead_counts_;
+    ap.ah.prod_block0 = 0;
+    ap.ah.prod_blocks = (int32_t)ahead_step_blocks_;
+    ap.ah.prod_pairs = (int32_t)ahead_step_pairs_;
+    ap.seed = m_.seed; ap.iter = ahead_step_iter_ + 1;
+    ap.n_local = sh_.n_local; ap.cap = sh_.cap; ap.gid0 = sh_.gid0;
+    ap.kind = ahead_producer_kind(m_.model_id, m_.s);
+  }
+  ahead_step_pending_ = false;
   if (pending_rows_ >= 0 && np_ <= 64 && pending_rows_ * np_ <= fuse_reduce_max_) {
     const int64_t rows = pending_rows_;
     pending_rows_ = -1;
     pending_xchg_ = false;
     prof_begin(SABC_KERNEL_REDUCE);
     HB_LAUNCH(launch_reduce_control(partials_, rows, np_, sums_stage_, pending_guarded_, cb_dev_, a, hist_dev_, mbox_dev_, stream_,
-                                    xchg ? &pv : nullptr, xchg ? tag(++xseq_) : 0, true, xchg ? take_silence() : 0),
+                                    xchg ? &pv : nullptr, xchg ? tag(++xseq_) : 0, true, xchg ? take_silence() : 0, &ap),
               "k_reduce_control");
     prof_end(SABC_KERNEL_REDUCE);
     return 0;
@@ -884,6 +982,7 @@
 }
 
 int HipBackend::upload(const double *theta, const double *u, const double *rho) {
+  if (ahead_clear()) return -1;
   const size_t w = (size_t)sh_.n_local * sizeof(double), pitch = (size_t)sh_.cap * sizeof(double);
   if (sh_.n_local > 0) {
     if (theta) HB_CHECK(hipMemcpy2DAsync(pop_[cur_], pitch, theta, w, w, (size_t)m_.d, hipMemcpyHostToDevice, stream_), "upload theta");
diff --git a/simulatedannealingabc.jl_amd/csrc/hip_backend.hpp b/simulatedannealingabc.jl_amd/csrc/hip_backend.hpp
--- a/simulatedannealingabc.jl_amd/csrc/hip_backend.hpp
+++ b/simulatedannealingabc.jl_amd/csrc/hip_backend.hpp
@@ -90,6 +90,7 @@
   void p2p_inject_silence(int n) { p2p_loss_ = false; if (n >= 0) { p2p_skip_ = 0; p2p_silent_ = n; } else { p2p_skip_ = -n; p2p_silent_ = 1; } }
   void p2p_inject_loss(int n) { p2p_loss_ = true; p2p_skip_ = n > 0 ? n : 0; p2p_silent_ = 1; }
   int64_t kernel_launches() const { return launches_; }
+  int64_t ahead_blocks(int which);
   double host_callback_seconds() const { return host_cb_seconds_; }
   int64_t host_callback_calls() const { return host_cb_calls_; }
   void set_host_chunk(int64_t particles) { host_chunk_ = particles > 0 ? particles : 0; }
@@ -218,6 +219,20 @@
   double *p2p_test_dev_ = nullptr;
   double *snap_pop_ = nullptr, *snap_rho_ = nullptr;
   int64_t launches_ = 0;
+  int ahead_alloc();
+  int ahead_clear();
+  bool ahead_update_args(const StepArgs &c, int64_t lo, int64_t cnt, int64_t rows, AheadArgs *out);
+  double *ahead_sums_[2] = {nullptr, nullptr};
+  unsigned long long *ahead_tags_[2] = {nullptr, nullptr};
+  unsigned long long *ahead_counts_ = nullptr;
+  int64_t ahead_n_blocks_ = 0, ahead_tag_words_ = 0;
+  int64_t ahead_a_ = -1, ahead_pairs_ = -1, ahead_fill_ = 0;
+  int cu_count_ = 256;
+  bool ahead_step_pending_ = false;
+  uint64_t ahead_step_iter_ = 0;
+  int64_t ahead_step_blocks_ = 0, ahead_step_pairs_ = 0;
+  int64_t ahead_covered_[2] = {0, 0};
+  uint64_t ahead_covered_iter_[2] = {0, 0};
   int64_t persist_max_ = 65536;
   unsigned long long *persist_sync_ = nullptr;
   unsigned long long *persist_rows_ = nullptr;
diff --git a/simulatedannealingabc.jl_amd/csrc/kernels.hip b/simulatedannealingabc.jl_amd/csrc/kernels.hip
--- a/simulatedannealingabc.jl_amd/csrc/kernels.hip
+++ b/simulatedannealingabc.jl_amd/csrc/kernels.hip
@@ -657,10 +657,27 @@
 #define RC_MARK(i) do { } while (0)
 #endif
 
-template <bool XCHG>
+template <int PROD>
+__device__ __forceinline__ void reduce_control_producer(const AheadProd &ap) {
+  rng_tables_load();
+  __syncthreads();
+  if (threadIdx.x >= kAheadBlock) return;
+  const int64_t t = (int64_t)(blockIdx.x - 1) * kAheadBlock + threadIdx.x;
+  if constexpr (PROD == 1) ahead_produce<SABC_MODEL_GAUSS_IID, 1, 1>(ap.seed, ap.ah, ap.iter, t, ap.n_local, ap.cap, ap.gid0);
+  else if constexpr (PROD == 2) ahead_produce<SABC_MODEL_GAUSS_IID, 1, 2>(ap.seed, ap.ah, ap.iter, t, ap.n_local, ap.cap, ap.gid0);
+  else if constexpr (PROD == 3) ahead_produce<SABC_MODEL_GAUSS2D, 2, 3>(ap.seed, ap.ah, ap.iter, t, ap.n_local, ap.cap, ap.gid0);
+}
+
+template <bool XCHG, int PROD = 0>
 __global__ void __launch_bounds__(1024)
 k_reduce_control(const double *__restrict__ partials, const int64_t rows, const int np, double *__restrict__ stage,
-                 ControlBlock *cb, const ControlArgs a, double *hist, Mailbox *ring, const XchgArgs x) {
+                 ControlBlock *cb, const ControlArgs a, double *hist, Mailbox *ring, const XchgArgs x, const AheadProd ap) {
+  if constexpr (PROD > 0) {
+    if (blockIdx.x > 0) {
+      if (!((a.mode & CTRL_GUARDED) && cb->halt)) reduce_control_producer<PROD>(ap);
+      return;
+    }
+  }
   __shared__ ControlBlock lcb;
   __shared__ int ran;
   __shared__ int failed;
@@ -1589,7 +1606,8 @@
                   int64_t act_lo, int64_t act_n, double *partials, int64_t row0, hipStream_t stream, hipEvent_t ev0,
                   hipEvent_t ev1, const RtcKernels *rtc) {
   if (act_n <= 0) return 0;
-  const dim3 grid((unsigned)update_rows(m, act_n)), block(m.model_id == SABC_MODEL_GK ? kBlock : update_block_threads(m.s));
+  const unsigned fill = c.ahead.sums[0] ? (unsigned)(((int64_t)c.ahead.prod_blocks * kAheadBlock + update_block_threads(m.s) - 1) / update_block_threads(m.s)) : 0u;
+  const dim3 grid((unsigned)update_rows(m, act_n) + fill), block(m.model_id == SABC_MODEL_GK ? kBlock : update_block_threads(m.s));
   double *out = partials + row0 * n_partials(m.d, m.s);
   if (m.model_id == SABC_MODEL_USER) {
     if (!rtc || c.prop_kind < 0 || c.prop_kind > 2 || !rtc->update[c.prop_kind]) return (int)hipErrorInvalidValue;
@@ -1684,18 +1702,29 @@
 
 int launch_reduce_control(const double *partials, int64_t rows, int np, double *stage, bool reduce_guarded,
                           ControlBlock *cb, const ControlArgs &a, double *hist, Mailbox *mbox, hipStream_t stream,
-                          const P2PView *pv, uint32_t seq, bool do_control, int silent) {
+                          const P2PView *pv, uint32_t seq, bool do_control, int silent, const AheadProd *ahead) {
   (void)reduce_guarded;
   XchgArgs x;
   std::memset(&x, 0, sizeof(x));
   x.do_control = do_control ? 1 : 0;
   static const int forced = [] { const char *e = std::getenv("SABC_RC_BLOCK"); const int v = e ? std::atoi(e) : 0; return (v == 256 || v == 1024) ? v : 0; }();
   const int block = forced && np <= 256 ? forced : ((rows < 0 && np <= 256) || (np <= 64 && rows >= 0 && rows <= (int64_t)24 * (256 / np))) ? 256 : 1024;
+  AheadProd ap;
+  std::memset(&ap, 0, sizeof(ap));
   if (pv) {
     x.pv = *pv; x.seq = seq; x.silent = silent;
-    hipLaunchKernelGGL(k_reduce_control<true>, dim3(1), dim3(block), 0, stream, partials, rows, np, stage, cb, a, hist, mbox, x);
+    hipLaunchKernelGGL(k_reduce_control<true>, dim3(1), dim3(block), 0, stream, partials, rows, np, stage, cb, a, hist, mbox, x, ap);
+  } else if (ahead && ahead->kind > 0 && ahead->ah.prod_blocks > 0) {
+    ap = *ahead;
+    const dim3 grid(1u + (unsigned)ap.ah.prod_blocks);
+    switch (ap.kind) {
+      case 1: hipLaunchKernelGGL((k_reduce_control<false, 1>), grid, dim3(block), 0, stream, partials, rows, np, stage, cb, a, hist, mbox, x, ap); break;
+      case 2: hipLaunchKernelGGL((k_reduce_control<false, 2>), grid, dim3(block), 0, stream, partials, rows, np, stage, cb, a, hist, mbox, x, ap); break;
+      case 3: hipLaunchKernelGGL((k_reduce_control<false, 3>), grid, dim3(block), 0, stream, partials, rows, np, stage, cb, a, hist, mbox, x, ap); break;
+      default: return (int)hipErrorInvalidValue;
+    }
   } else {
-    hipLaunchKernelGGL(k_reduce_control<false>, dim3(1), dim3(block), 0, stream, partials, rows, np, stage, cb, a, hist, mbox, x);
+    hipLaunchKernelGGL(k_reduce_control<false>, dim3(1), dim3(block), 0, stream, partials, rows, np, stage, cb, a, hist, mbox, x, ap);
   }
   return SABC_LAUNCH_RC();
 }
diff --git a/simulatedannealingabc.jl_amd/csrc/kernels.hpp b/simulatedannealingabc.jl_amd/csrc/kernels.hpp
--- a/simulatedannealingabc.jl_amd/csrc/kernels.hpp
+++ b/simulatedannealingabc.jl_amd/csrc/kernels.hpp
@@ -90,6 +90,20 @@
          (long)update_block_threads(s) * 8 + (long)sizeof(ControlBlock) + (long)kMaxPartials * 8 + 2048 <= 156 * 1024;
 }
 
+constexpr int ahead_producer_kind(int model, int s) {
+  return model == SABC_MODEL_GAUSS_IID ? (s >= 2 ? 2 : 1) : model == SABC_MODEL_GAUSS2D ? 3 : 0;
+}
+constexpr int ahead_sums_per_particle(int model, int s) {
+  return model == SABC_MODEL_GAUSS_IID ? (s >= 2 ? 2 : 1) : model == SABC_MODEL_GAUSS2D ? 5 : 0;
+}
+constexpr bool update_carries_producers(int model, int s) { return !(model == SABC_MODEL_GAUSS_IID && s >= 2); }
+struct AheadProd {
+  AheadArgs ah;
+  uint64_t seed, iter;
+  int64_t n_local, cap, gid0;
+  int32_t kind, reserved;
+};
+
 #if !defined(__HIPCC_RTC__)
 int launch_prior_simulate(const ModelDesc &m, PopPtrs pp, hipStream_t stream, const RtcKernels *rtc = nullptr);
 int launch_cdf_population(const ModelDesc &m, PopPtrs pp, CdfPtrs cdf, hipStream_t stream);
@@ -111,7 +125,8 @@
                    hipStream_t stream);
 int launch_reduce_control(const double *partials, int64_t rows, int np, double *stage, bool reduce_guarded,
                           ControlBlock *cb, const ControlArgs &a, double *hist, Mailbox *mbox, hipStream_t stream,
-                          const P2PView *pv = nullptr, uint32_t seq = 0, bool do_control = true, int silent = 0);
+                          const P2PView *pv = nullptr, uint32_t seq = 0, bool do_control = true, int silent = 0,
+                          const AheadProd *ahead = nullptr);
 int launch_p2p_barrier(const P2PView &pv, uint32_t seq, ControlBlock *cb, bool guarded, int silent, hipStream_t stream);
 int launch_p2p_commit(const P2PView &pv, uint32_t call, int status, bool wait, ControlBlock *cb, int silent, hipStream_t stream);
 int launch_p2p_selftest(const P2PView &pv, uint32_t seq, int np, const double *in, double *out, int *failed, int silent,
diff --git a/simulatedannealingabc.jl_amd/csrc/rtc.cpp b/simulatedannealingabc.jl_amd/csrc/rtc.cpp
--- a/simulatedannealingabc.jl_amd/csrc/rtc.cpp
+++ b/simulatedannealingabc.jl_amd/csrc/rtc.cpp
@@ -203,6 +203,7 @@
                 "\nnamespace sabc {\n"
                 "template <int D, int S>\n"
                 "struct Sim<SABC_MODEL_USER, D, S> {\n"
+                "  static constexpr int kAheadSums = 0;\n"
                 "  static __device__ __forceinline__ void run(const ModelDesc &m, const double *th, uint64_t pid, uint64_t iter,\n"
                 "                                             double *rho, int coop = 0) {\n"
                 "    NormalStream ns(m.seed, pid, PURPOSE_SIM, iter, coop);\n"
diff --git a/simulatedannealingabc.jl_amd/csrc/sabc_types.hpp b/simulatedannealingabc.jl_amd/csrc/sabc_types.hpp
--- a/simulatedannealingabc.jl_amd/csrc/sabc_types.hpp
+++ b/simulatedannealingabc.jl_amd/csrc/sabc_types.hpp
@@ -27,10 +27,22 @@
   uint64_t seed;
 };
 
+constexpr int kAheadBlock = 256;
+constexpr int kAheadPairBits = 20;
+struct AheadArgs {
+  double *sums[2];
+  unsigned long long *tags[2];
+  unsigned long long *counts;
+  int32_t own_blocks;
+  int32_t prod_block0, prod_blocks;
+  int32_t prod_pairs;
+};
+
 struct StepArgs {
   uint64_t iter;
   int32_t prop_kind, reserved;
   double prop_p0, prop_p1;
+  AheadArgs ahead;
 };
 
 struct ControlBlock {
diff --git a/simulatedannealingabc.jl_amd/csrc/update_kernel.hpp b/simulatedannealingabc.jl_amd/csrc/update_kernel.hpp
--- a/simulatedannealingabc.jl_amd/csrc/update_kernel.hpp
+++ b/simulatedannealingabc.jl_amd/csrc/update_kernel.hpp
@@ -107,6 +107,45 @@
   else *p = v;
 }
 
+struct AheadIn {
+  const double *sums = nullptr;
+  bool have = false;
+  int first = 0;
+};
+template <int MODEL, int D, int S, int PROP, int LANES, bool ONE_LAUNCH>
+constexpr bool ahead_consumer() {
+  return Sim<MODEL, D, S>::kAheadSums > 0 && PROP == SABC_PROP_RANDOMWALK && LANES == 1 && !ONE_LAUNCH;
+}
+
+__device__ __forceinline__ int ahead_lookup(const AheadArgs &ah, const uint64_t iter, const int64_t p0) {
+  const int b = __builtin_amdgcn_readfirstlane((int)(p0 / kAheadBlock));
+  const unsigned long long tag = ah.tags[iter & 1][b];
+  const bool hit = (tag >> kAheadPairBits) == iter + 1;
+  return __builtin_amdgcn_readfirstlane(hit ? (int)(tag & ((1ull << kAheadPairBits) - 1)) : -1);
+}
+
+template <int MODEL, int D, int S>
+__device__ __forceinline__ void ahead_produce(const uint64_t seed, const AheadArgs &ah, const uint64_t iter, const int64_t t,
+                                              const int64_t n_local, const int64_t cap, const int64_t gid0) {
+  using M = Sim<MODEL, D, S>;
+  if constexpr (M::kAheadSums > 0) {
+    const int64_t p = (int64_t)ah.prod_block0 * kAheadBlock + t;
+    const int64_t b = p / kAheadBlock;
+    if (b >= (int64_t)ah.prod_block0 + ah.prod_blocks || p >= n_local) return;
+    double sums[M::kAheadSums];
+#pragma unroll
+    for (int a = 0; a < M::kAheadSums; ++a) sums[a] = 0.0;
+    M::draw(seed, (uint64_t)(gid0 + p), iter, 0, ah.prod_pairs, sums, update_loop_coop(MODEL, D, S, SABC_PROP_RANDOMWALK, false));
+    double *out = ah.sums[iter & 1];
+#pragma unroll
+    for (int a = 0; a < M::kAheadSums; ++a) out[(int64_t)a * cap + p] = sums[a];
+    if (p % kAheadBlock == 0) {
+      ah.tags[iter & 1][b] = ((unsigned long long)(iter + 1) << kAheadPairBits) | (unsigned long long)ah.prod_pairs;
+      atomicAdd(ah.counts, 1ull);
+    }
+  }
+}
+
 template <int D, int S>
 struct ParticleDraft {
   double th[D], u[S];
@@ -117,7 +156,7 @@
 template <int MODEL, int D, int S, int PROP, bool PAST_CACHES, int LANES, bool ONE_LAUNCH = false, class CB>
 __device__ __forceinline__ void update_particle_draft(const ModelDesc &m, const uint64_t iter, const double prop_p0, const double prop_p1,
                                                       const CB *__restrict__ cb, const PopPtrs &pp, const PartnerView &pv, const int64_t li,
-                                                      const uint64_t gid, ParticleDraft<D, S> &q) {
+                                                      const uint64_t gid, ParticleDraft<D, S> &q, const AheadIn &ahead = AheadIn()) {
 #pragma unroll
   for (int k = 0; k < D; ++k) q.th[k] = pp.pop[(int64_t)k * pp.cap + li];
 #pragma unroll
@@ -173,7 +212,15 @@
 #pragma unroll
   for (int j = 0; j < S; ++j) q.rp[j] = 0.0;
   if (q.lpp > -INFINITY) {
-    if (LANES > 1) Sim<MODEL, D, S>::run(m, q.thp, gid, iter, q.rp, LANES);
+    if constexpr (ahead_consumer<MODEL, D, S, PROP, LANES, ONE_LAUNCH>()) {
+      using M = Sim<MODEL, D, S>;
+      double sums[M::kAheadSums];
+#pragma unroll
+      for (int a = 0; a < M::kAheadSums; ++a) sums[a] = ahead.have ? ahead.sums[(int64_t)a * pp.cap + li] : 0.0;
+      const int coop = update_loop_coop(MODEL, D, S, PROP, ONE_LAUNCH);
+      M::draw(m.seed, gid, iter, ahead.first, M::loop_pairs(m) - ahead.first, sums, coop);
+      M::finish(m, q.thp, gid, iter, sums, q.rp, coop);
+    } else if (LANES > 1) Sim<MODEL, D, S>::run(m, q.thp, gid, iter, q.rp, LANES);
     else Sim<MODEL, D, S>::run(m, q.thp, gid, iter, q.rp, update_loop_coop(MODEL, D, S, PROP, ONE_LAUNCH));
   }
   SABC_TRACE(iter, 8);
@@ -237,9 +284,9 @@
 __device__ __forceinline__ void update_particle(const ModelDesc &m, const uint64_t iter, const double prop_p0, const double prop_p1,
                                                 const CB *__restrict__ cb, const PopPtrs &pp, const CdfPtrs &cdf, const PartnerView &pv,
                                                 const double (&cidx)[S][cdf_coarse_entries(S)], const int64_t li, const uint64_t gid,
-                                                double (&acc)[n_partials(D, S)]) {
+                                                double (&acc)[n_partials(D, S)], const AheadIn &ahead = AheadIn()) {
   ParticleDraft<D, S> q;
-  update_particle_draft<MODEL, D, S, PROP, PAST_CACHES, LANES, LATENCY>(m, iter, prop_p0, prop_p1, cb, pp, pv, li, gid, q);
+  update_particle_draft<MODEL, D, S, PROP, PAST_CACHES, LANES, LATENCY>(m, iter, prop_p0, prop_p1, cb, pp, pv, li, gid, q, ahead);
   update_particle_decide<D, S, PAST_CACHES, LANES, LATENCY>(m, iter, cb, pp, cdf, cidx, li, gid, q, acc);
 }
 
@@ -251,6 +298,15 @@
   if (cb->halt) return;
   rng_tables_load();
   constexpr int kUpdateBlock = update_block_threads(S), kCoarse = cdf_coarse_entries(S);
+  constexpr bool kAhead = ahead_consumer<MODEL, D, S, PROP, 1, false>();
+  if constexpr (kAhead && update_carries_producers(MODEL, S)) {
+    if (c.ahead.sums[0] && (int)blockIdx.x >= c.ahead.own_blocks) {
+      __syncthreads();
+      ahead_produce<MODEL, D, S>(m.seed, c.ahead, c.iter + 1, (int64_t)((int)blockIdx.x - c.ahead.own_blocks) * kUpdateBlock + threadIdx.x,
+                                 pp.n_local, pp.cap, pp.gid0);
+      return;
+    }
+  }
   __shared__ double cidx[S][kCoarse];
   load_coarse_index<S>(cdf, cidx);
   __syncthreads();
@@ -259,9 +315,21 @@
   for (int q = 0; q < NP; ++q) acc[q] = 0.0;
 
   const int64_t t = (int64_t)blockIdx.x * kUpdateBlock + threadIdx.x;
+  AheadIn ahead;
+  if constexpr (kAhead) {
+    if (c.ahead.sums[0]) {
+      const int first = ahead_lookup(c.ahead, c.iter, (int64_t)blockIdx.x * kUpdateBlock + (threadIdx.x & ~63u));
+      if (first >= 0) {
+        ahead.sums = c.ahead.sums[c.iter & 1];
+        ahead.have = true;
+        ahead.first = first;
+        if (t % kAheadBlock == 0 && t < act_n) atomicAdd(c.ahead.counts + 1, 1ull);
+      }
+    }
+  }
   if (t < act_n) {
     const int64_t li = act_lo + t;
-    update_particle<MODEL, D, S, PROP>(m, c.iter, c.prop_p0, c.prop_p1, cb, pp, cdf, pv, cidx, li, (uint64_t)(pp.gid0 + li), acc);
+    update_particle<MODEL, D, S, PROP>(m, c.iter, c.prop_p0, c.prop_p1, cb, pp, cdf, pv, cidx, li, (uint64_t)(pp.gid0 + li), acc, ahead);
   }
   block_reduce_store<NP, kUpdateBlock>(acc, partials + (int64_t)blockIdx.x * NP);
 }
@@ -341,6 +409,7 @@
 constexpr int kDraftOnly = -1;
 template <int D, int S>
 struct Sim<kDraftOnly, D, S> {
+  static constexpr int kAheadSums = 0;
   static __device__ __forceinline__ void run(const ModelDesc &, const double *, uint64_t, uint64_t, double *, int = 0) {}
 };
 
diff --git a/simulatedannealingabc.jl_amd/handle.py b/simulatedannealingabc.jl_amd/handle.py
--- a/simulatedannealingabc.jl_amd/handle.py
+++ b/simulatedannealingabc.jl_amd/handle.py
@@ -312,6 +312,14 @@
         return int(self._L.sabc_kernel_launches(self._h))
 
     @property
+    def ahead_blocks_produced(self):
+        return int(self._L.sabc_ahead_blocks(self._h, 0))
+
+    @property
+    def ahead_blocks_consumed(self):
+        return int(self._L.sabc_ahead_blocks(self._h, 1))
+
+    @property
     def collective_calls(self):
         return int(self._L.sabc_collective_calls(self._h))
 
```

Result: slower. 6.499 billion (-1.0%).
